# osmocom/osmo-trx

Measured on AMD Instinct MI355X. Metric: Mbursts/s detect+demod (156.25 sym, 4 SPS), higher is better.
Workload: dtype f32

## Files before the change

osmo_trx_amd/csrc/trx_kernel_nb.hip:

```cpp
#include "trx_k4_common.h"
#include "trx_nb_asm.inc"

#define NB_D_LEN    160
#define NB_CZ_LEN   (TRX_CZ_PAD + TRX_CORR_NARROW + TRX_CZ_PAD)
#define NB_SLICE    (K4_XS + NB_D_LEN + NB_CZ_LEN)
#define NB_COMP_ROWS (TRX_DELAY_FILTS + 1)
#define NB_TABLES_FLOATS (TRX_SINCV_LDS + 16 * WAVE + NB_COMP_ROWS * 36 + 16 + 8 * 8 + 5 * WAVE + 5 * WAVE + 2 * 8 * 16)
#define NB_TABLES_BYTES (NB_TABLES_FLOATS * 4)
#define NB_WPB 16
#define NB_POOL_RING 64
#define NB_POOL_UNSET (-1)
#define NB_POOL_END (-2)
#define NB_NO_BURST 0xffffffffu
#define NB_LDS_TAIL (16 + 4 * NB_POOL_RING)
#define NB_LDS_BYTES (NB_TABLES_BYTES + NB_WPB * NB_SLICE * 8 + NB_LDS_TAIL)
#define NB_MAX_TOA 32



typedef float v3f __attribute__((ext_vector_type(3)));
typedef int v4i __attribute__((ext_vector_type(4)));
typedef __attribute__((address_space(3))) v2f lds_v2f;

template <typename T>
__device__ __forceinline__ unsigned lds_addr(const T *p)
{
	return (unsigned)(uintptr_t)(const __attribute__((address_space(3))) T *)p;
}

__device__ __forceinline__ int nb_lane_id()
{
	int lane;
	asm volatile("v_mbcnt_lo_u32_b32 %0, -1, 0\n\tv_mbcnt_hi_u32_b32 %0, -1, %0" : "=v"(lane));
	return lane;
}

__global__ void __launch_bounds__(NB_WPB * WAVE)
nb_pull4_kernel(const uint32_t *__restrict__ iq, const trxhip_burst_params *__restrict__ params,
		trxhip_burst_result *__restrict__ results, float *__restrict__ soft, const trx_tables *__restrict__ tab,
		unsigned n_bursts, float thresh, float full_scale, unsigned *__restrict__ pool_ctr, unsigned *__restrict__ redo,
		float gk5, float gk6, float gk7, float gk8)
{
	static_assert(NB_TABLES_BYTES % 16 == 0 && (NB_SLICE * 8) % 16 == 0 && (K4_XS * 8) % 16 == 0 && (NB_D_LEN * 8) % 16 == 0, "16-byte LDS accesses");
	static_assert(NB_LDS_BYTES <= 160 * 1024, "LDS");
	static_assert(NB_ASM_GDEC_OFF == (TRX_SINCV_LDS + 16 * WAVE + NB_COMP_ROWS * 36) * 4, "tools/gen_nb_asm.py: LDS offset of the decimator taps");
	static_assert(NB_ASM_DEC_MAX_NACT == 15 + NB_ASM_CORR_MAX_LEN, "tools/gen_nb_asm.py: DEC and CORR change form at the same window (one test)");
	static_assert(NB_ASM_LSEQ_OFF == (NB_TABLES_FLOATS - 2 * 8 * 16) * 4, "tools/gen_nb_asm.py: LDS offset of the training-sequence taps");
	static_assert(NB_ASM_AW_PD == (PH_M0 + 52) * 8 && NB_ASM_AW_D == K4_XS * 8 && NB_ASM_AW_CZ == (K4_XS + NB_D_LEN + TRX_CZ_PAD) * 8,
		      "tools/gen_nb_asm.py: offsets of P, D[] and cz[] inside a wave's slice");
	constexpr int NLD = 10;
	extern __shared__ __attribute__((aligned(16))) char smem[];
	const int lane0 = threadIdx.x & (WAVE - 1);
	const int wave = uni((int)(threadIdx.x >> 6));

	float *const sincv = reinterpret_cast<float *>(smem);
	float *const wa4f = sincv + TRX_SINCV_LDS;
	const float4 *const wa4 = reinterpret_cast<const float4 *>(wa4f);
	float *const comp = wa4f + 16 * WAVE;
	float *const gdec = comp + NB_COMP_ROWS * 36;
	float *const lhdr = gdec + 16;
	int *const pkcl = reinterpret_cast<int *>(lhdr + 8 * 8);
	int *const lcn = pkcl + 5 * WAVE;
	c32 *const lseq = reinterpret_cast<c32 *>(lcn + 5 * WAVE);
	c32 *const wbase = reinterpret_cast<c32 *>(smem + NB_TABLES_BYTES) + (size_t)wave * NB_SLICE;
	int *const wg_next = reinterpret_cast<int *>(reinterpret_cast<c32 *>(smem + NB_TABLES_BYTES) + (size_t)NB_WPB * NB_SLICE);
	int *const pool_g = wg_next + 4;
	c32 *const P = wbase;
	c32 *const D = wbase + K4_XS;
	c32 *const cz = D + NB_D_LEN + TRX_CZ_PAD;

	for (int i = threadIdx.x; i < TRX_SINCV_LDS; i += blockDim.x)
		sincv[i] = (i < TRX_SINCV_LEN) ? tab->sincv[i] : 0.0f;
	for (int i = threadIdx.x; i < 16 * WAVE; i += blockDim.x) {
		const int l = i & (WAVE - 1), u = i >> 6;
		const PeakConst pcl = peak_const(l);
		const int q = (u < 8) ? pcl.loA + 512 * (7 - u) : pcl.hiA + 512 * (u - 8);
		wa4f[((u >> 2) * WAVE + l) * 4 + (u & 3)] = (q < TRX_SINCV_LEN) ? tab->sincv[q] : 0.0f;
	}
	for (int i = threadIdx.x; i < NB_COMP_ROWS * 36; i += blockDim.x) {
		const int f = i / 36, j = i % 36;
		comp[i] = (j >= TRX_FUSED_SH) ? tab->comp_filt[f][j - TRX_FUSED_SH] : 0.0f;
	}
	if (threadIdx.x < 16)
		gdec[threadIdx.x] = tab->dec_taps[threadIdx.x];
	if (threadIdx.x < 128)
		lseq[threadIdx.x] = make_float2(tab->seq[TRX_SEQ_TSC0 + (threadIdx.x >> 4)].taps[threadIdx.x & 15].re,
						tab->seq[TRX_SEQ_TSC0 + (threadIdx.x >> 4)].taps[threadIdx.x & 15].im);
	if (threadIdx.x < 64)
		lhdr[threadIdx.x] = reinterpret_cast<const float *>(&tab->seq[TRX_SEQ_TSC0 + (threadIdx.x >> 3)].gain)[threadIdx.x & 7];
	if (threadIdx.x < WAVE) {
		const PeakConst pc0 = peak_const(threadIdx.x);
		pkcl[0 * WAVE + threadIdx.x] = pc0.flA;
		pkcl[1 * WAVE + threadIdx.x] = pc0.loA;
		pkcl[2 * WAVE + threadIdx.x] = pc0.hiA;
		pkcl[3 * WAVE + threadIdx.x] = pc0.offB;
		pkcl[4 * WAVE + threadIdx.x] = pc0.ratio_off;
		lcn[0 * WAVE + threadIdx.x] = pc0.ratio_off * 8;
		lcn[1 * WAVE + threadIdx.x] = (pc0.flA - 8) * 8;
		lcn[2 * WAVE + threadIdx.x] = pc0.offB;
		const int l = threadIdx.x, e = (l - 52) / 3, t = (l - 52) % 3;
		const bool sp = l >= 52;
		lcn[3 * WAVE + l] = 8 * (sp ? (t == 0 ? e : t == 1 ? e + 3 : e - 3) : 4 + 3 * (l < 49 ? l : 49));
		lcn[4 * WAVE + l] = sp ? (e + (t == 2 ? 4 : 0)) * K4_NTP * 4 : -1;
	}
	for (int i = lane0; i < NB_SLICE; i += WAVE)
		wbase[i] = make_float2(0.0f, 0.0f);
	if (threadIdx.x == 0) {
		wg_next[0] = NB_WPB;
		wg_next[1] = 0;
	}
	if (threadIdx.x < NB_POOL_RING)
		pool_g[threadIdx.x] = NB_POOL_UNSET;
	__syncthreads();

	const float thr2 = thresh * thresh;
	float gkv = lane0 == 5 ? gk5 : lane0 == 6 ? gk6 : lane0 == 7 ? gk7 : gk8;
	asm volatile("" : "+v"(gkv));
	const float gc0 = thr2 * 1.0001e-5f;
	int t5pk = 0;
	bool t5_ok = true;
	for (int t = 0; t < 8; t++) {
		const int v = (int)(lhdr[8 * t + 5] * 512.0f);
		t5_ok = t5_ok && v >= -8 && v <= 7 && (float)v == lhdr[8 * t + 5] * 512.0f;
		t5pk |= (v & 15) << (4 * t);
	}
	t5pk = uni(t5pk);
	const unsigned toa_lim = (unsigned)uni(t5_ok ? (int)((NB_MAX_TOA + 1u) << 16) : 0);
	const unsigned long long e8_addr = reinterpret_cast<unsigned long long>(&tab->edge8[0][0][0]);
	const unsigned n_wg = gridDim.x;
	const unsigned n_groups = (n_bursts + 15u) >> 4;
	const bool pooled = pool_ctr != nullptr;
	const unsigned n_static_groups = pooled ? ((n_groups - (n_groups >> 3)) / n_wg) * n_wg : n_groups;
	const unsigned n_pool_groups = n_groups - n_static_groups;
	const unsigned gq = n_static_groups / n_wg, gr = n_static_groups % n_wg;
	const unsigned my_groups = gq + (blockIdx.x < gr ? 1u : 0u);
	const unsigned base16 = (blockIdx.x * gq + (blockIdx.x < gr ? blockIdx.x : gr)) << 4;
	unsigned items = my_groups << 4;
	if (base16 + items > n_bursts)
		items = (base16 < n_bursts) ? n_bursts - base16 : 0u;
	auto burst_of = [&](unsigned jj) -> unsigned {
		if (__builtin_expect(jj < items, 1))
			return base16 + jj;
		if (!pooled)
			return NB_NO_BURST;
		const unsigned k = (jj - items) >> 4;
		volatile int *slot = pool_g + (k & (NB_POOL_RING - 1));
		int g;
		while ((g = *slot) == NB_POOL_UNSET)
			__builtin_amdgcn_s_sleep(2);
		g = uni(g);
		if (g < 0)
			return NB_NO_BURST;
		const unsigned bb = ((n_static_groups + (unsigned)g) << 4) + (jj & 15u);
		return bb < n_bursts ? bb : NB_NO_BURST;
	};
	auto pool_draw = [&](unsigned jj, bool ended) {
		const int lane = nb_lane_id();
		const unsigned k = (jj + 16u - items) >> 4;
		int g = NB_POOL_END;
		if (!ended) {
			unsigned p = 0;
			if (lane == 0)
				p = __hip_atomic_fetch_add(pool_ctr, 1u, __ATOMIC_RELAXED, __HIP_MEMORY_SCOPE_AGENT);
			p = (unsigned)uni((int)p);
			g = (p < n_pool_groups) ? (int)p : NB_POOL_END;
		}
		if (lane == 0) {
			pool_g[(k + NB_POOL_RING / 2) & (NB_POOL_RING - 1)] = NB_POOL_UNSET;
			pool_g[k & (NB_POOL_RING - 1)] = g;
		}
	};

	unsigned a_p = lds_addr(wbase) + 8u * (unsigned)((lane0 & 3) * PH_A + PH_M0 + (lane0 >> 2));
	unsigned a_w = lds_addr(wbase) + 8u * (unsigned)lane0;
	unsigned a_l4 = 4u * (unsigned)lane0;
	unsigned a_l4c = 4u * min((unsigned)lane0, 48u);
	unsigned a_l16 = 16u * (unsigned)lane0;
	unsigned a_st = (lane0 >= 54) ? 4u * (unsigned)((lane0 - 54) / 3) : (unsigned)(lane0 - 2) * 12u + 16u;
	asm volatile("" : "+v"(a_p));
	asm volatile("" : "+v"(a_w));
	asm volatile("" : "+v"(a_l4));
	asm volatile("" : "+v"(a_l4c));
	asm volatile("" : "+v"(a_l16));
	asm volatile("" : "+v"(a_st));

	uint32_t pre_i[NLD];
	uint32_t pre_prm = 0u;
	auto prefetch = [&](unsigned bb) {
		pre_prm = reinterpret_cast<const uint32_t *>(params)[2 * (size_t)bb];
		const char *src = reinterpret_cast<const char *>(iq + (size_t)bb * 625);
		const uint32_t *const row = reinterpret_cast<const uint32_t *>(src + a_l4);
#pragma unroll
		for (int r = 0; r < NLD - 1; r++)
			pre_i[r] = __builtin_nontemporal_load(row + r * WAVE);
		pre_i[NLD - 1] = __builtin_nontemporal_load(reinterpret_cast<const uint32_t *>(src + a_l4c) + (NLD - 1) * WAVE);
	};
	const unsigned b_first = burst_of((unsigned)wave);
	if (b_first != NB_NO_BURST)
		prefetch(b_first);

	v3f o = { 0.0f, 0.0f, 0.0f };
	int recw = 0;
	int pend_m = 0;
	int pend_rm = 0;
	unsigned pend_b = 0;
	int left_any = 0;
	auto store_pending = [&]() {
		float *const so = soft + (size_t)pend_b * 148;
		int *const rp = reinterpret_cast<int *>(results + pend_b);
		const float oe = o.x;
		asm volatile("s_bfm_b64 exec, 48, 2\n\t"
			     "s_and_b32 exec_lo, exec_lo, %7\n\t"
			     "s_and_b32 exec_hi, exec_hi, %7\n\t"
			     "global_store_dwordx3 %0, %1, %2\n\t"
			     "s_mov_b32 exec_lo, 0\n\t"
			     "s_and_b32 exec_hi, %7, 0x92400000\n\t"
			     "global_store_dword %0, %3, %2\n\t"
			     "s_mov_b32 exec_lo, %8\n\t"
			     "s_mov_b32 exec_hi, 0\n\t"
			     "global_store_dword %4, %5, %6\n\t"
			     "s_mov_b64 exec, -1\n\t"
			     "s_nop 0"
			     :: "v"(a_st), "v"(o), "s"(so), "v"(oe), "v"(a_l4), "v"(recw), "s"(rp), "s"(pend_m), "s"(pend_rm)
			     : "memory", "scc");
	};
	int q_xr = 0, q_xi = 0, q_es = 0, q_toa = 0, q_s = 0, q_fl = 0, q_b = 0;
	int q_n = 0;
	auto flush_records = [&]() {
		const int lane = nb_lane_id();
		if (lane < q_n) {
			const float *const h = lhdr + 8 * (q_fl & 0xff);
			const float xr = __int_as_float(q_xr), xi = __int_as_float(q_xi);
			const float a0 = xr * h[2], a1 = xr * h[3], a2 = xi * h[3], a3 = xi * h[2];
			const float amp_re = a0 - a2, amp_im = a1 + a3;
			const float toa = (float)q_toa * 0.001953125f;
			const float energy = __int_as_float(q_es) * 0.0125f;
			const float rssi = rssi_db(full_scale, energy);
			const float p2 = xi * xi + xr * xr;
			const float C = p2 * h[7];
			const float S = __int_as_float(q_s);
			const float ci = 3.0103f * __log2f(C * __builtin_amdgcn_rcpf(S - C));
			const v4i r0 = { 1, __float_as_int(toa), __float_as_int(amp_re), __float_as_int(amp_im) };
			const v4i r1 = { __float_as_int(ci), __float_as_int(energy), __float_as_int(rssi), q_fl };
			asm volatile("global_store_dwordx4 %0, %1, off\n\t"
				     "global_store_dwordx4 %0, %2, off offset:16\n\t"
				     "s_nop 1"
				     :: "v"(results + (unsigned)q_b), "v"(r0), "v"(r1) : "memory");
		}
		asm volatile("");
		q_n = 0;
	};

	auto queue_record = [&](const int xr_bits, const int xi_bits, const int es_bits, const int toa, const int s_bits, const int fl, const unsigned bb) {
		asm("s_lshl_b64 exec, 1, %[n]\n\t"
		    "v_mov_b32_e32 %[qxr], %[xr]\n\t"
		    "v_mov_b32_e32 %[qxi], %[xi]\n\t"
		    "v_mov_b32_e32 %[qes], %[es]\n\t"
		    "v_mov_b32_e32 %[qtoa], %[toa]\n\t"
		    "v_mov_b32_e32 %[qs], %[ss]\n\t"
		    "v_mov_b32_e32 %[qfl], %[fl]\n\t"
		    "v_mov_b32_e32 %[qb], %[b]\n\t"
		    "s_mov_b64 exec, -1"
		    : [qxr] "+v"(q_xr), [qxi] "+v"(q_xi), [qes] "+v"(q_es), [qtoa] "+v"(q_toa), [qs] "+v"(q_s), [qfl] "+v"(q_fl),
		      [qb] "+v"(q_b)
		    : [n] "s"(uni(q_n)), [xr] "s"(xr_bits), [xi] "s"(xi_bits), [es] "s"(es_bits), [toa] "s"(toa),
		      [ss] "s"(s_bits), [fl] "s"(fl), [b] "s"((int)bb)
		    : "scc");
		q_n++;
	};

	auto demod_general = [&](const int nk, const c32 ampv, const int lane) -> bool {
		constexpr int L = 625, nwrite = 148;
		c32 *const dec = D;
		const trx_tables *tabc = reinterpret_cast<const trx_tables *>(e8_addr - offsetof(trx_tables, edge8));
		asm volatile("" : "+s"(tabc));
		const int w = nk >> 7, fr = nk & 127;
		const int fidx = (fr >= 2) ? (fr >> 1) : TRX_DELAY_FILTS;
		const float ian = __builtin_amdgcn_rcpf(norm2(ampv));
		const c32 scale = make_float2(ampv.x * ian, -ampv.y * ian);
		const int n_lo = w > 0 ? w : 0;
		const int n_hi = (L - 1 + w < 623) ? L - 1 + w : 623;
		const int i_full_lo = cdiv4(n_lo + 15), i_full_hi = fdiv4(n_hi);
		const int i0l = cdiv4(n_lo), i0h = i_full_hi + 1;
		const bool need_lo = (n_hi >= n_lo) && (i0l < i_full_lo) && (i0l < nwrite);
		const bool need_hi = (n_hi >= n_lo) && (i0h <= fdiv4(n_hi + 15)) && (i0h < nwrite);
		if (uni((need_lo && !(n_hi >= 4 * (i_full_lo - 1))) || (need_hi && !((w <= -2) && (n_lo <= 4 * i0h - 15)))))
			return false;
		const int lo_tab = uni(need_lo);
		float ct0 = 0.0f, ct1 = 0.0f, ct2 = 0.0f;
		const int le = lane >> 4, lt = lane & 15;
		const int li = i0l + le;
		const int lt0 = n_lo + 15 - 4 * li;
		const bool lact = lt0 >= 1;
		if (lo_tab) {
			const float *row = &tabc->edge_lo[fidx][(lact ? lt0 : 1) - 1][lt];
			ct0 = row[0];
			ct1 = row[16];
			ct2 = (lt < 4) ? row[32] : 0.0f;
		}
		const int hi_tab = uni(need_hi);
		float ch0 = 0.0f, ch1 = 0.0f, ch2 = 0.0f;
		const int hi_i = i0h + le;
		const int htm = n_hi + 15 - 4 * hi_i;
		const bool hact = htm >= 0;
		if (hi_tab) {
			const float *row = &tabc->edge_hi[fidx][hact ? htm : 0][lt];
			ch0 = row[0];
			ch1 = row[16];
			ch2 = (lt < 4) ? row[32] : 0.0f;
		}
		int tabv = lo_tab | (hi_tab << 1);
		asm volatile("" : "+v"(tabv));
		{
			const int c_full = -24 - w;
			const int i_min = cdiv4(-36 - c_full), i_max = fdiv4(L + 1 - c_full);
			int ic = 3 * lane;
			if (ic < i_min) ic = i_min;
			if (ic > i_max - 2) ic = i_max - 2;
			v2f acc[3];
			asm volatile(NB_ASM_FIRG
				     : [a0] "=&v"(acc[0]), [a1] "=&v"(acc[1]), [a2] "=&v"(acc[2])
				     : [nk] "s"(nk), [pb] "s"(lds_addr(P)), [cb] "s"(lds_addr(comp) + 4u * (K4_U0 + TRX_FUSED_SH)), [kic] "v"(8 * ic)
				     : NB_ASM_CLOBBERS);
			if (n_lo == 0 && lo_tab && i_full_hi >= nwrite - 1) {
				if (lane < 52) {
#pragma unroll
					for (int j = 0; j < 3; j++)
						dec[3 * lane + j] = cmul(make_float2(acc[j].x, acc[j].y), scale);
				}
			} else {
#pragma unroll
				for (int j = 0; j < 3; j++) {
					const int i = 3 * lane + j;
					const bool full = (i >= i_full_lo) && (i <= i_full_hi);
					const c32 d = full ? cmul(make_float2(acc[j].x, acc[j].y), scale) : make_float2(0.0f, 0.0f);
					if (i < 156)
						dec[i] = d;
				}
			}
		}
		const int tab2 = uni(tabv), lo_tab2 = tab2 & 1, hi_tab2 = tab2 & 2;
		if (lo_tab2) {
			const int s0 = 4 * li - 24 - w + lt;
			const c32 *pp = P + ((s0 & 3) * PH_A + PH_M0 + (s0 >> 2));
			const c32 x0 = lds_c32(pp), x1 = lds_c32(pp + 4), x2 = lds_c32(pp + 8);
			float ar = x0.x * ct0, ai = x0.y * ct0;
			ar = fmaf(x1.x, ct1, ar); ai = fmaf(x1.y, ct1, ai);
			ar = fmaf(x2.x, ct2, ar); ai = fmaf(x2.y, ct2, ai);
			const float sr = row_sum(ar), si = row_sum(ai);
			int lt0s = lt0;
			asm volatile("" : "+v"(lt0s));
			if (lt == 0 && lt0s >= 1)
				dec[li] = cmul(make_float2(sr, si), scale);
		}
		if (hi_tab2) {
			const int s0 = 4 * hi_i - 24 - w + lt;
			const c32 *pp = P + ((s0 & 3) * PH_A + PH_M0 + (s0 >> 2));
			const c32 x0 = lds_c32(pp), x1 = lds_c32(pp + 4), x2 = lds_c32(pp + 8);
			float ar = x0.x * ch0, ai = x0.y * ch0;
			ar = fmaf(x1.x, ch1, ar); ai = fmaf(x1.y, ch1, ai);
			ar = fmaf(x2.x, ch2, ar); ai = fmaf(x2.y, ch2, ai);
			const float sr = row_sum(ar), si = row_sum(ai);
			int htms = htm;
			asm volatile("" : "+v"(htms));
			if (lt == 0 && htms >= 0 && hi_i < 156)
				dec[hi_i] = cmul(make_float2(sr, si), scale);
		}
		wave_sync();
		auto pick = [&](int i) {
			const float d = reinterpret_cast<const float *>(dec + i)[i & 1];
			return __builtin_amdgcn_fmed3f(fmaf((i & 2) ? -0.5f : 0.5f, d, 0.5f), 0.0f, 1.0f);
		};
		const bool reg = lane >= 2 && lane < 50;
		const int i0 = reg ? 3 * lane - 2 : ((((lane - 54) * 11) >> 5) & 3);
		o.x = pick(i0);
		o.y = pick(reg ? i0 + 1 : 0);
		o.z = pick(reg ? i0 + 2 : 0);
		wave_sync();
		return true;
	};

	DIAG_DECL;
	unsigned j_next = 0, b_next = NB_NO_BURST;
	const unsigned j_plain = (unsigned)uni((int)(!pooled ? items : items >= 16u ? items - 16u : 0u));
	auto advance = [&](const int taken) {
		j_next = (unsigned)taken;
		if (__builtin_expect(j_next < j_plain, 1)) {
			b_next = base16 + j_next;
			DIAG_MARK(17);
			prefetch(b_next);
		} else {
			b_next = burst_of(j_next);
			if (pooled && (j_next & 15u) == 0u && j_next + 16u >= items)
				pool_draw(j_next, b_next == NB_NO_BURST && j_next >= items);
			DIAG_MARK(17);
			if (b_next != NB_NO_BURST)
				prefetch(b_next);
		}
	};
	auto mark_left = [&](const unsigned bb) {
		if (nb_lane_id() == 0) {
			reinterpret_cast<uint8_t *>(redo + TRX_REDO_HDR)[bb] = 1;
			if (!left_any)
				__hip_atomic_store(redo, 1u, __ATOMIC_RELAXED, __HIP_MEMORY_SCOPE_AGENT);
		}
		asm volatile("");
		left_any = 1;
	};
	for (unsigned b = b_first; __builtin_expect(b != NB_NO_BURST, 1); b = b_next) {
		asm volatile("" : "+v"(a_l4));
		asm volatile("" : "+v"(a_l4c));
		const int ticket = claim_issue(wg_next);
		const unsigned prm0 = (unsigned)uni((int)pre_prm);
		const unsigned max_toa = prm0 >> 16;
		const int tsc = (prm0 >> 8) & 0xff;
#ifdef TRX_DIAG
		DIAG_MARK(12);
		asm volatile("s_waitcnt vmcnt(0)" ::: "memory");
		DIAG_MARK(13);
#endif
		const unsigned slot_key = prm0 | (0u - ((prm0 & 0xf8ffu) ^ (unsigned)TRXHIP_TSC));
		int keep = -1;
		if (__builtin_expect(slot_key >= toa_lim, 0)) {
#pragma unroll
			for (int r = 0; r < NLD; r++)
				asm volatile("" :: "v"(pre_i[r]));
			store_pending();
			advance(claim_take(ticket));
			pend_rm = 0;
			mark_left(b);
			keep = 0;
		} else {
			lds_v2f *const pload = reinterpret_cast<lds_v2f *>(a_p);
			float amax = 0.0f, epart = 0.0f;
#pragma unroll
			for (int r = 0; r < NLD; r++) {
				const v2f v = { (float)(int16_t)(pre_i[r] & 0xffffu), (float)(int16_t)(pre_i[r] >> 16) };
				if (r < NLD - 1)
					pload[16 * r] = v;
				else
					asm volatile("s_bfm_b64 exec, 49, 0\n\t"
						     "ds_write_b64 %0, %1 offset:%c2\n\t"
						     "s_mov_b64 exec, -1"
						     :: "v"(a_p), "v"(v), "n"(128 * (NLD - 1)) : "memory");
				asm("v_max3_f32 %0, %0, |%1|, |%2|" : "+v"(amax) : "v"(v.x), "v"(v.y));
				if (r < 5)
					epart = fmaf(v.x, v.x, fmaf(v.y, v.y, epart));
			}
			DIAG_MARK(14);
			store_pending();
			DIAG_MARK(16);
			advance(claim_take_behind<5>(ticket));
			DIAG_MARK(15);

			pend_rm = 0;
			{
				int clip;
				asm("s_cmp_lg_u64 %1, 0\n\ts_cselect_b32 %0, 1, 0" : "=s"(clip) : "s"(__ballot(amax > TRX_CLIP_THRESH)) : "scc");

				const int len = 16 + (int)max_toa;
				__builtin_assume(len >= 16 && len <= 16 + NB_MAX_TOA);
				float v;
				const int lag0 = (len <= NB_ASM_CORR_MAX_LEN) ? NB_ASM_CORR_LANE0 : 0;
				asm volatile(NB_ASM_DECCORR
					     : [nrm] "=&v"(v)
					     : [aw] "v"(a_w), [zero] "v"(0), [len] "s"(len), [tsc] "s"(tsc)
					     : NB_ASM_CLOBBERS);
				{
					DIAG_MARK(3);
					int m_bits, es_bits, bidx;
					int kr, ka, kb, kic, ktp;
					asm volatile(NB_ASM_AMAX("ds_read_b32 %[kr], %[l4] offset:%c[lc]", "ds_read_b32 %[ka], %[l4] offset:%c[lc]+256",
								 "ds_read_b32 %[kb], %[l4] offset:%c[lc]+512", "ds_read_b32 %[kic], %[l4] offset:%c[lc]+768",
								 "ds_read_b32 %[ktp], %[l4] offset:%c[lc]+1024", "s_nop 0", "s_nop 0", "s_nop 0")
						     "s_sub_u32 %[bidx], %[bidx], %[lag0]\n\t"
						     "s_waitcnt lgkmcnt(0)"
						     : [m] "=&s"(m_bits), [es] "=&s"(es_bits), [bidx] "=&s"(bidx), [kr] "=&v"(kr), [ka] "=&v"(ka), [kb] "=&v"(kb),
						       [kic] "=&v"(kic), [ktp] "=&v"(ktp)
						     : [nrm] "v"(v), [ep] "v"(epart), [l4] "v"(a_l4), [lag0] "s"(lag0),
						       [lc] "n"((TRX_SINCV_LDS + 16 * WAVE + NB_COMP_ROWS * 36 + 16 + 64 + 5 * WAVE) * 4)
						     : NB_ASM_CLOBBERS);
					DIAG_MARK(4);
					int st, e512;
					float km;
					asm volatile(NB_ASM_DETA
						     : [st] "=&" NB_ASM_ST(st), [e] "=&s"(e512), [km] "=&v"(km)
						     : [bidx] "s"(bidx), [len] "s"(len), [czb] "s"(lds_addr(cz)), [kr] "v"(kr), [ka] "v"(ka), [l16] "v"(a_l16),
						       [gkv] "v"(gkv), [c0] "v"(gc0)
						     : NB_ASM_CLOBBERS_ST);
					DIAG_MARK(5);
					int toa512 = 0, xr_bits = 0, xi_bits = 0;
					if (__builtin_expect(st == 1, 1)) {
						asm volatile(NB_ASM_DETB
							     : [st] "=&" NB_ASM_ST(st), [toa] "=&s"(toa512), [xr] "=&s"(xr_bits), [xi] "=&s"(xi_bits)
							     : [e] "s"(e512), [kb] "v"(kb), [czb] "s"(lds_addr(cz)), [km] "v"(km)
							     : NB_ASM_CLOBBERS_ST);
						DIAG_MARK(6);
					}
					if (__builtin_expect(st != 1, 0)) {
						int stc = st;
						asm volatile("" : "+s"(stc));
						if (stc == 3) {
							const int lane = nb_lane_id();
							if (lane == 0)
								atomicAdd(&g_trx_fast_stats[0], 1ull);
							PeakConst pkc;
							pkc.flA = pkcl[0 * WAVE + lane]; pkc.loA = pkcl[1 * WAVE + lane]; pkc.hiA = pkcl[2 * WAVE + lane];
							pkc.offB = pkcl[3 * WAVE + lane]; pkc.ratio_off = pkcl[4 * WAVE + lane];
							c32 xcorr;
							peak_detect_spec(cz, bidx, sincv, pkc, lane, &toa512, &xcorr, wa4);
							toa512 = uni(toa512);
							xr_bits = uni(__float_as_int(xcorr.x));
							xi_bits = uni(__float_as_int(xcorr.y));
							st = 1;
						} else if (stc == 2) {
							if (nb_lane_id() == 0) atomicAdd(&g_trx_fast_stats[2], 1ull);
							mark_left(b);
							keep = 0;
						} else {
							const float energy = __int_as_float(es_bits) * 0.0125f;
							const float rssi = rssi_db(full_scale, energy);
							const uint32_t flags = ((uint32_t)clip << 8) | (1u << 16);
							int word = clip ? -TRXHIP_SIGERR_CLIP : 0;
							word = put_lane<1>(word, 0.0f);
							word = put_lane<2>(word, 0.0f);
							word = put_lane<3>(word, 0.0f);
							word = put_lane<4>(word, 0.0f);
							word = put_lane<5>(word, energy);
							word = put_lane<6>(word, rssi);
							word = write_lane<7>(word, (int)flags);
							recw = word;
							o = (v3f){ 0.0f, 0.0f, 0.0f };
							pend_rm = 0xff;
						}
					}
					if (__builtin_expect(st == 1, 1)) {
						int ok, s_bits;
						float d0, d1, d2;
						const int t5 = (t5pk << (28 - 4 * tsc)) >> 28;
						asm volatile("s_setprio 0");
						asm volatile(NB_ASM_TAIL
							     : [ok] "=&s"(ok), [ssum] "=&s"(s_bits), [d0] "=&v"(d0), [d1] "=&v"(d1), [d2] "=&v"(d2)
							     : [toa] "s"(toa512), [xr] "s"(xr_bits), [xi] "s"(xi_bits), [t5] "s"(t5), [hdrb] "s"(lds_addr(lhdr) + 32u * (unsigned)tsc),
							       [e8lo] "s"((unsigned)e8_addr), [e8hi] "s"((unsigned)(e8_addr >> 32)), [l16] "v"(a_l16),
							       [aw] "v"(a_w), [pb] "s"(lds_addr(P)), [cb] "s"(lds_addr(comp) + 4u * (K4_U0 + TRX_FUSED_SH)), [db] "s"(lds_addr(D)),
							       [kic] "v"(kic), [ktp] "v"(ktp)
							     : NB_ASM_CLOBBERS);
						DIAG_MARK(10);
						asm volatile("s_setprio 2");
						o.x = __builtin_amdgcn_fmed3f(fmaf(0.5f, d0, 0.5f), 0.0f, 1.0f);
						o.y = __builtin_amdgcn_fmed3f(fmaf(0.5f, d1, 0.5f), 0.0f, 1.0f);
						o.z = __builtin_amdgcn_fmed3f(fmaf(0.5f, d2, 0.5f), 0.0f, 1.0f);
						queue_record(xr_bits, xi_bits, es_bits, toa512 - t5 - 10 * 512, s_bits,
							     (int)((uint32_t)tsc | ((uint32_t)clip << 8) | (37u << 24)), b);
						if (__builtin_expect(!ok, 0)) {
							const int lane = nb_lane_id();
							if (lane == 0) atomicAdd(&g_trx_fast_stats[3], 1ull);
							const float *const h = lhdr + 8 * tsc;
							const float xr = __int_as_float(xr_bits), xi = __int_as_float(xi_bits);
							const float a0 = xr * h[2], a1 = xr * h[3], a2 = xi * h[3], a3 = xi * h[2];
							const c32 ampv = make_float2(unif(a0 - a2), unif(a1 + a3));
							if (!demod_general(t5 + 10 * 512 - toa512, ampv, lane)) {
								q_n--;
								mark_left(b);
								keep = 0;
							}
						}
					}
				}
			}
		}
		pend_b = b;
		pend_m = keep;
		if (__builtin_expect(q_n == WAVE, 0))
			flush_records();
		DIAG_MARK(11);
	}
	asm volatile(NB_ASM_COLD ::: NB_ASM_CLOBBERS);
	store_pending();
	flush_records();
	DIAG_FLUSH();
	if (pooled) {
		__syncthreads();
		int tid0;
		asm volatile("v_mbcnt_lo_u32_b32 %0, -1, 0\n\tv_mbcnt_hi_u32_b32 %0, -1, %0" : "=v"(tid0));
		if (tid0 == 0 && atomicAdd(wg_next + 1, 1) == 0) {
			const unsigned d = __hip_atomic_fetch_add(pool_ctr + 1, 1u, __ATOMIC_ACQ_REL, __HIP_MEMORY_SCOPE_AGENT);
			if (d == gridDim.x - 1u) {
				__hip_atomic_store(pool_ctr, 0u, __ATOMIC_RELAXED, __HIP_MEMORY_SCOPE_AGENT);
				__hip_atomic_store(pool_ctr + 1, 0u, __ATOMIC_RELEASE, __HIP_MEMORY_SCOPE_AGENT);
			}
		}
	}
}
```

osmo_trx_amd/csrc/trx_nb_asm.inc:

```
#define NB_ASM_GDEC_OFF 29968
#define NB_ASM_LSEQ_OFF 32848
#define NB_ASM_DEC_MAX_NACT 60
#define NB_ASM_CORR_LANE0 19
#define NB_ASM_CORR_MAX_LEN 45
#define NB_ASM_AW_PD 512
#define NB_ASM_AW_D 5760
#define NB_ASM_AW_CZ 7136
#define NB_ASM_ST "{s98}"
#define NB_ASM_CLOBBERS "v64", "v65", "v66", "v67", "v68", "v69", "v70", "v71", "v72", "v73", "v74", "v75", "v76", "v77", "v78", "v79", "v80", "v81", "v82", "v83", "v84", "v85", "v86", "v87", "v88", "v89", "v90", "v91", "v92", "v93", "v94", "v95", "v96", "v97", "v98", "v99", "v100", "v101", "v102", "v103", "v104", "v105", "v106", "v107", "v108", "v109", "v110", "v111", "v112", "v113", "v114", "v115", "v116", "v117", "v118", "v119", "v120", "v121", "v122", "v123", "v124", "v125", "v126", "v127", "s87", "s88", "s89", "s90", "s91", "s92", "s93", "s94", "s95", "s96", "s97", "s98", "s99", "vcc", "scc", "memory"
#define NB_ASM_CLOBBERS_ST "v64", "v65", "v66", "v67", "v68", "v69", "v70", "v71", "v72", "v73", "v74", "v75", "v76", "v77", "v78", "v79", "v80", "v81", "v82", "v83", "v84", "v85", "v86", "v87", "v88", "v89", "v90", "v91", "v92", "v93", "v94", "v95", "v96", "v97", "v98", "v99", "v100", "v101", "v102", "v103", "v104", "v105", "v106", "v107", "v108", "v109", "v110", "v111", "v112", "v113", "v114", "v115", "v116", "v117", "v118", "v119", "v120", "v121", "v122", "v123", "v124", "v125", "v126", "v127", "s87", "s88", "s89", "s90", "s91", "s92", "s93", "s94", "s95", "s96", "s97", "s99", "vcc", "scc", "memory"
#define NB_ASM_DECCORR \
	"s_add_u32 s92, %[len], 15\n\t" \
	"s_cmp_gt_u32 %[len], 45\n\t" \
	"s_cbranch_scc1 .Lnbc_dc_wide\n\t" \
	"s_sub_u32 s88, 60, s92\n\t" \
	"s_lshr_b64 exec, -1, s88\n\t" \
	"ds_read_b128 v[120:123], %[zero] offset:29968\n\t" \
	"ds_read_b128 v[124:127], %[zero] offset:29984\n\t" \
	"ds_read_b64 v[98:99], %[aw] offset:1952\n\t" \
	"ds_read_b64 v[100:101], %[aw] offset:3392\n\t" \
	"ds_read_b64 v[102:103], %[aw] offset:4832\n\t" \
	"ds_read_b64 v[96:97], %[aw] offset:512\n\t" \
	"s_waitcnt lgkmcnt(3)\n\t" \
	"v_pk_mul_f32 v[64:65], v[98:99], v[120:121] op_sel:[0,0] op_sel_hi:[1,0]\n\t" \
// ... 880 lines not shown
	"v_add_f32_dpp v121, v121, v110 wave_shr:1 row_mask:0xf bank_mask:0xf bound_ctrl:0\n\t" \
	"s_nop 0\n\t" \
	"v_add_f32_dpp v120, v120, v110 wave_shr:1 row_mask:0xf bank_mask:0xf bound_ctrl:0\n\t" \
	"v_add_f32_dpp v121, v121, v111 wave_shr:1 row_mask:0xf bank_mask:0xf bound_ctrl:0\n\t" \
	"s_nop 0\n\t" \
	"v_sub_f32_dpp v120, v120, v111 wave_shr:1 row_mask:0xf bank_mask:0xf bound_ctrl:0\n\t" \
	"v_add_f32_dpp v121, v121, v110 wave_shr:1 row_mask:0xf bank_mask:0xf bound_ctrl:0\n\t" \
	"s_nop 0\n\t" \
	"v_sub_f32_dpp v120, v120, v110 wave_shr:1 row_mask:0xf bank_mask:0xf bound_ctrl:0\n\t" \
	"v_sub_f32_dpp v121, v121, v111 wave_shr:1 row_mask:0xf bank_mask:0xf bound_ctrl:0\n\t" \
	"s_nop 0\n\t" \
	"v_add_f32_dpp v120, v120, v111 wave_shr:1 row_mask:0xf bank_mask:0xf bound_ctrl:0\n\t" \
	"v_sub_f32_dpp v121, v121, v110 wave_shr:1 row_mask:0xf bank_mask:0xf bound_ctrl:0\n\t" \
	"s_nop 0\n\t" \
	"v_sub_f32_dpp v120, v120, v110 wave_shr:1 row_mask:0xf bank_mask:0xf bound_ctrl:0\n\t" \
	"v_sub_f32_dpp v121, v121, v111 wave_shr:1 row_mask:0xf bank_mask:0xf bound_ctrl:0\n\t" \
	"s_nop 0\n\t" \
	"v_sub_f32_dpp v120, v120, v111 wave_shr:1 row_mask:0xf bank_mask:0xf bound_ctrl:0\n\t" \
	"v_add_f32_dpp v121, v121, v110 wave_shr:1 row_mask:0xf bank_mask:0xf bound_ctrl:0\n\t" \
	"s_nop 0\n\t" \
	"v_sub_f32_dpp v120, v120, v110 wave_shr:1 row_mask:0xf bank_mask:0xf bound_ctrl:0\n\t" \
	"v_sub_f32_dpp v121, v121, v111 wave_shr:1 row_mask:0xf bank_mask:0xf bound_ctrl:0\n\t" \
	"s_nop 0\n\t" \
	"v_add_f32_dpp v120, v120, v111 wave_shr:1 row_mask:0xf bank_mask:0xf bound_ctrl:0\n\t" \
	"v_sub_f32_dpp v121, v121, v110 wave_shr:1 row_mask:0xf bank_mask:0xf bound_ctrl:0\n\t" \
	"s_nop 0\n\t" \
	"v_sub_f32_dpp v120, v120, v110 wave_shr:1 row_mask:0xf bank_mask:0xf bound_ctrl:0\n\t" \
	"v_sub_f32_dpp v121, v121, v111 wave_shr:1 row_mask:0xf bank_mask:0xf bound_ctrl:0\n\t" \
	"s_nop 0\n\t" \
	"v_sub_f32_dpp v120, v120, v111 wave_shr:1 row_mask:0xf bank_mask:0xf bound_ctrl:0\n\t" \
	"v_add_f32_dpp v121, v121, v110 wave_shr:1 row_mask:0xf bank_mask:0xf bound_ctrl:0\n\t" \
	"s_bfm_b64 exec, 12, 0\n\t" \
	"ds_write_b64 v64, v[122:123] offset:7136\n\t" \
	"s_bfm_b64 exec, %[len], 19\n\t" \
	"ds_write_b64 %[aw], v[120:121] offset:6984\n\t" \
	"v_pk_mul_f32 v[124:125], v[120:121], v[120:121]\n\t" \
	"s_nop 0\n\t" \
	"v_add_f32_e32 %[nrm], v125, v124\n\t" \
	"s_mov_b64 exec, -1\n\t" \
	"s_waitcnt lgkmcnt(0)\n\t" \
	"s_branch .Lnb_corr_end\n\t" \
	".Lnb_corrr_v4:\n\t" \
	"v_add_f32_e32 v120, 0, v110\n\t" \
	"v_add_f32_e32 v121, 0, v111\n\t" \
	"s_nop 0\n\t" \
	"v_sub_f32_dpp v120, v120, v111 wave_shr:1 row_mask:0xf bank_mask:0xf bound_ctrl:0\n\t" \
	"v_add_f32_dpp v121, v121, v110 wave_shr:1 row_mask:0xf bank_mask:0xf bound_ctrl:0\n\t" \
	"s_nop 0\n\t" \
	"v_sub_f32_dpp v120, v120, v110 wave_shr:1 row_mask:0xf bank_mask:0xf bound_ctrl:0\n\t" \
	"v_sub_f32_dpp v121, v121, v111 wave_shr:1 row_mask:0xf bank_mask:0xf bound_ctrl:0\n\t" \
	"s_nop 0\n\t" \
	"v_add_f32_dpp v120, v120, v111 wave_shr:1 row_mask:0xf bank_mask:0xf bound_ctrl:0\n\t" \
	"v_sub_f32_dpp v121, v121, v110 wave_shr:1 row_mask:0xf bank_mask:0xf bound_ctrl:0\n\t" \
	"s_nop 0\n\t" \
	"v_sub_f32_dpp v120, v120, v110 wave_shr:1 row_mask:0xf bank_mask:0xf bound_ctrl:0\n\t" \
	"v_sub_f32_dpp v121, v121, v111 wave_shr:1 row_mask:0xf bank_mask:0xf bound_ctrl:0\n\t" \
	"s_nop 0\n\t" \
	"v_sub_f32_dpp v120, v120, v111 wave_shr:1 row_mask:0xf bank_mask:0xf bound_ctrl:0\n\t" \
	"v_add_f32_dpp v121, v121, v110 wave_shr:1 row_mask:0xf bank_mask:0xf bound_ctrl:0\n\t" \
	"s_nop 0\n\t" \
	"v_sub_f32_dpp v120, v120, v110 wave_shr:1 row_mask:0xf bank_mask:0xf bound_ctrl:0\n\t" \
	"v_sub_f32_dpp v121, v121, v111 wave_shr:1 row_mask:0xf bank_mask:0xf bound_ctrl:0\n\t" \
	"s_nop 0\n\t" \
	"v_sub_f32_dpp v120, v120, v111 wave_shr:1 row_mask:0xf bank_mask:0xf bound_ctrl:0\n\t" \
	"v_add_f32_dpp v121, v121, v110 wave_shr:1 row_mask:0xf bank_mask:0xf bound_ctrl:0\n\t" \
	"s_nop 0\n\t" \
	"v_sub_f32_dpp v120, v120, v110 wave_shr:1 row_mask:0xf bank_mask:0xf bound_ctrl:0\n\t" \
	"v_sub_f32_dpp v121, v121, v111 wave_shr:1 row_mask:0xf bank_mask:0xf bound_ctrl:0\n\t" \
	"s_nop 0\n\t" \
	"v_add_f32_dpp v120, v120, v111 wave_shr:1 row_mask:0xf bank_mask:0xf bound_ctrl:0\n\t" \
	"v_sub_f32_dpp v121, v121, v110 wave_shr:1 row_mask:0xf bank_mask:0xf bound_ctrl:0\n\t" \
	"s_nop 0\n\t" \
	"v_sub_f32_dpp v120, v120, v110 wave_shr:1 row_mask:0xf bank_mask:0xf bound_ctrl:0\n\t" \
	"v_sub_f32_dpp v121, v121, v111 wave_shr:1 row_mask:0xf bank_mask:0xf bound_ctrl:0\n\t" \
	"s_nop 0\n\t" \
	"v_sub_f32_dpp v120, v120, v111 wave_shr:1 row_mask:0xf bank_mask:0xf bound_ctrl:0\n\t" \
	"v_add_f32_dpp v121, v121, v110 wave_shr:1 row_mask:0xf bank_mask:0xf bound_ctrl:0\n\t" \
	"s_nop 0\n\t" \
	"v_add_f32_dpp v120, v120, v110 wave_shr:1 row_mask:0xf bank_mask:0xf bound_ctrl:0\n\t" \
	"v_add_f32_dpp v121, v121, v111 wave_shr:1 row_mask:0xf bank_mask:0xf bound_ctrl:0\n\t" \
	"s_nop 0\n\t" \
	"v_add_f32_dpp v120, v120, v111 wave_shr:1 row_mask:0xf bank_mask:0xf bound_ctrl:0\n\t" \
	"v_sub_f32_dpp v121, v121, v110 wave_shr:1 row_mask:0xf bank_mask:0xf bound_ctrl:0\n\t" \
	"s_nop 0\n\t" \
	"v_add_f32_dpp v120, v120, v110 wave_shr:1 row_mask:0xf bank_mask:0xf bound_ctrl:0\n\t" \
	"v_add_f32_dpp v121, v121, v111 wave_shr:1 row_mask:0xf bank_mask:0xf bound_ctrl:0\n\t" \
	"s_nop 0\n\t" \
	"v_add_f32_dpp v120, v120, v111 wave_shr:1 row_mask:0xf bank_mask:0xf bound_ctrl:0\n\t" \
	"v_sub_f32_dpp v121, v121, v110 wave_shr:1 row_mask:0xf bank_mask:0xf bound_ctrl:0\n\t" \
	"s_bfm_b64 exec, 12, 0\n\t" \
	"ds_write_b64 v64, v[122:123] offset:7136\n\t" \
	"s_bfm_b64 exec, %[len], 19\n\t" \
	"ds_write_b64 %[aw], v[120:121] offset:6984\n\t" \
	"v_pk_mul_f32 v[124:125], v[120:121], v[120:121]\n\t" \
	"s_nop 0\n\t" \
	"v_add_f32_e32 %[nrm], v125, v124\n\t" \
	"s_mov_b64 exec, -1\n\t" \
	"s_waitcnt lgkmcnt(0)\n\t" \
	"s_branch .Lnb_corr_end\n\t" \
	".Lnb_corrr_v5:\n\t" \
	"v_sub_f32_e32 v120, 0, v110\n\t" \
	"v_sub_f32_e32 v121, 0, v111\n\t" \
	"s_nop 0\n\t" \
	"v_sub_f32_dpp v120, v120, v111 wave_shr:1 row_mask:0xf bank_mask:0xf bound_ctrl:0\n\t" \
	"v_add_f32_dpp v121, v121, v110 wave_shr:1 row_mask:0xf bank_mask:0xf bound_ctrl:0\n\t" \
	"s_nop 0\n\t" \
	"v_sub_f32_dpp v120, v120, v110 wave_shr:1 row_mask:0xf bank_mask:0xf bound_ctrl:0\n\t" \
	"v_sub_f32_dpp v121, v121, v111 wave_shr:1 row_mask:0xf bank_mask:0xf bound_ctrl:0\n\t" \
	"s_nop 0\n\t" \
	"v_add_f32_dpp v120, v120, v111 wave_shr:1 row_mask:0xf bank_mask:0xf bound_ctrl:0\n\t" \
	"v_sub_f32_dpp v121, v121, v110 wave_shr:1 row_mask:0xf bank_mask:0xf bound_ctrl:0\n\t" \
	"s_nop 0\n\t" \
	"v_add_f32_dpp v120, v120, v110 wave_shr:1 row_mask:0xf bank_mask:0xf bound_ctrl:0\n\t" \
	"v_add_f32_dpp v121, v121, v111 wave_shr:1 row_mask:0xf bank_mask:0xf bound_ctrl:0\n\t" \
	"s_nop 0\n\t" \
	"v_sub_f32_dpp v120, v120, v111 wave_shr:1 row_mask:0xf bank_mask:0xf bound_ctrl:0\n\t" \
	"v_add_f32_dpp v121, v121, v110 wave_shr:1 row_mask:0xf bank_mask:0xf bound_ctrl:0\n\t" \
	"s_nop 0\n\t" \
	"v_add_f32_dpp v120, v120, v110 wave_shr:1 row_mask:0xf bank_mask:0xf bound_ctrl:0\n\t" \
	"v_add_f32_dpp v121, v121, v111 wave_shr:1 row_mask:0xf bank_mask:0xf bound_ctrl:0\n\t" \
	"s_nop 0\n\t" \
	"v_sub_f32_dpp v120, v120, v111 wave_shr:1 row_mask:0xf bank_mask:0xf bound_ctrl:0\n\t" \
	"v_add_f32_dpp v121, v121, v110 wave_shr:1 row_mask:0xf bank_mask:0xf bound_ctrl:0\n\t" \
	"s_nop 0\n\t" \
	"v_add_f32_dpp v120, v120, v110 wave_shr:1 row_mask:0xf bank_mask:0xf bound_ctrl:0\n\t" \
	"v_add_f32_dpp v121, v121, v111 wave_shr:1 row_mask:0xf bank_mask:0xf bound_ctrl:0\n\t" \
	"s_nop 0\n\t" \
	"v_add_f32_dpp v120, v120, v111 wave_shr:1 row_mask:0xf bank_mask:0xf bound_ctrl:0\n\t" \
	"v_sub_f32_dpp v121, v121, v110 wave_shr:1 row_mask:0xf bank_mask:0xf bound_ctrl:0\n\t" \
	"s_nop 0\n\t" \
	"v_sub_f32_dpp v120, v120, v110 wave_shr:1 row_mask:0xf bank_mask:0xf bound_ctrl:0\n\t" \
	"v_sub_f32_dpp v121, v121, v111 wave_shr:1 row_mask:0xf bank_mask:0xf bound_ctrl:0\n\t" \
	"s_nop 0\n\t" \
	"v_sub_f32_dpp v120, v120, v111 wave_shr:1 row_mask:0xf bank_mask:0xf bound_ctrl:0\n\t" \
	"v_add_f32_dpp v121, v121, v110 wave_shr:1 row_mask:0xf bank_mask:0xf bound_ctrl:0\n\t" \
	"s_nop 0\n\t" \
	"v_sub_f32_dpp v120, v120, v110 wave_shr:1 row_mask:0xf bank_mask:0xf bound_ctrl:0\n\t" \
	"v_sub_f32_dpp v121, v121, v111 wave_shr:1 row_mask:0xf bank_mask:0xf bound_ctrl:0\n\t" \
	"s_nop 0\n\t" \
	"v_add_f32_dpp v120, v120, v111 wave_shr:1 row_mask:0xf bank_mask:0xf bound_ctrl:0\n\t" \
	"v_sub_f32_dpp v121, v121, v110 wave_shr:1 row_mask:0xf bank_mask:0xf bound_ctrl:0\n\t" \
	"s_nop 0\n\t" \
	"v_sub_f32_dpp v120, v120, v110 wave_shr:1 row_mask:0xf bank_mask:0xf bound_ctrl:0\n\t" \
	"v_sub_f32_dpp v121, v121, v111 wave_shr:1 row_mask:0xf bank_mask:0xf bound_ctrl:0\n\t" \
	"s_nop 0\n\t" \
	"v_add_f32_dpp v120, v120, v111 wave_shr:1 row_mask:0xf bank_mask:0xf bound_ctrl:0\n\t" \
	"v_sub_f32_dpp v121, v121, v110 wave_shr:1 row_mask:0xf bank_mask:0xf bound_ctrl:0\n\t" \
	"s_bfm_b64 exec, 12, 0\n\t" \
	"ds_write_b64 v64, v[122:123] offset:7136\n\t" \
	"s_bfm_b64 exec, %[len], 19\n\t" \
	"ds_write_b64 %[aw], v[120:121] offset:6984\n\t" \
	"v_pk_mul_f32 v[124:125], v[120:121], v[120:121]\n\t" \
	"s_nop 0\n\t" \
	"v_add_f32_e32 %[nrm], v125, v124\n\t" \
	"s_mov_b64 exec, -1\n\t" \
	"s_waitcnt lgkmcnt(0)\n\t" \
	"s_branch .Lnb_corr_end\n\t" \
	".Lnb_corrr_v6:\n\t" \
	"v_sub_f32_e32 v120, 0, v110\n\t" \
	"v_sub_f32_e32 v121, 0, v111\n\t" \
	"s_nop 0\n\t" \
	"v_sub_f32_dpp v120, v120, v111 wave_shr:1 row_mask:0xf bank_mask:0xf bound_ctrl:0\n\t" \
	"v_add_f32_dpp v121, v121, v110 wave_shr:1 row_mask:0xf bank_mask:0xf bound_ctrl:0\n\t" \
	"s_nop 0\n\t" \
	"v_add_f32_dpp v120, v120, v110 wave_shr:1 row_mask:0xf bank_mask:0xf bound_ctrl:0\n\t" \
	"v_add_f32_dpp v121, v121, v111 wave_shr:1 row_mask:0xf bank_mask:0xf bound_ctrl:0\n\t" \
	"s_nop 0\n\t" \
	"v_add_f32_dpp v120, v120, v111 wave_shr:1 row_mask:0xf bank_mask:0xf bound_ctrl:0\n\t" \
	"v_sub_f32_dpp v121, v121, v110 wave_shr:1 row_mask:0xf bank_mask:0xf bound_ctrl:0\n\t" \
	"s_nop 0\n\t" \
	"v_sub_f32_dpp v120, v120, v110 wave_shr:1 row_mask:0xf bank_mask:0xf bound_ctrl:0\n\t" \
	"v_sub_f32_dpp v121, v121, v111 wave_shr:1 row_mask:0xf bank_mask:0xf bound_ctrl:0\n\t" \
	"s_nop 0\n\t" \
	"v_add_f32_dpp v120, v120, v111 wave_shr:1 row_mask:0xf bank_mask:0xf bound_ctrl:0\n\t" \
	"v_sub_f32_dpp v121, v121, v110 wave_shr:1 row_mask:0xf bank_mask:0xf bound_ctrl:0\n\t" \
	"s_nop 0\n\t" \
	"v_add_f32_dpp v120, v120, v110 wave_shr:1 row_mask:0xf bank_mask:0xf bound_ctrl:0\n\t" \
	"v_add_f32_dpp v121, v121, v111 wave_shr:1 row_mask:0xf bank_mask:0xf bound_ctrl:0\n\t" \
	"s_nop 0\n\t" \
	"v_add_f32_dpp v120, v120, v111 wave_shr:1 row_mask:0xf bank_mask:0xf bound_ctrl:0\n\t" \
	"v_sub_f32_dpp v121, v121, v110 wave_shr:1 row_mask:0xf bank_mask:0xf bound_ctrl:0\n\t" \
	"s_nop 0\n\t" \
	"v_add_f32_dpp v120, v120, v110 wave_shr:1 row_mask:0xf bank_mask:0xf bound_ctrl:0\n\t" \
	"v_add_f32_dpp v121, v121, v111 wave_shr:1 row_mask:0xf bank_mask:0xf bound_ctrl:0\n\t" \
	"s_nop 0\n\t" \
	"v_add_f32_dpp v120, v120, v111 wave_shr:1 row_mask:0xf bank_mask:0xf bound_ctrl:0\n\t" \
	"v_sub_f32_dpp v121, v121, v110 wave_shr:1 row_mask:0xf bank_mask:0xf bound_ctrl:0\n\t" \
	"s_nop 0\n\t" \
	"v_sub_f32_dpp v120, v120, v110 wave_shr:1 row_mask:0xf bank_mask:0xf bound_ctrl:0\n\t" \
	"v_sub_f32_dpp v121, v121, v111 wave_shr:1 row_mask:0xf bank_mask:0xf bound_ctrl:0\n\t" \
	"s_nop 0\n\t" \
	"v_add_f32_dpp v120, v120, v111 wave_shr:1 row_mask:0xf bank_mask:0xf bound_ctrl:0\n\t" \
	"v_sub_f32_dpp v121, v121, v110 wave_shr:1 row_mask:0xf bank_mask:0xf bound_ctrl:0\n\t" \
	"s_nop 0\n\t" \
	"v_add_f32_dpp v120, v120, v110 wave_shr:1 row_mask:0xf bank_mask:0xf bound_ctrl:0\n\t" \
	"v_add_f32_dpp v121, v121, v111 wave_shr:1 row_mask:0xf bank_mask:0xf bound_ctrl:0\n\t" \
	"s_nop 0\n\t" \
	"v_sub_f32_dpp v120, v120, v111 wave_shr:1 row_mask:0xf bank_mask:0xf bound_ctrl:0\n\t" \
	"v_add_f32_dpp v121, v121, v110 wave_shr:1 row_mask:0xf bank_mask:0xf bound_ctrl:0\n\t" \
	"s_nop 0\n\t" \
	"v_sub_f32_dpp v120, v120, v110 wave_shr:1 row_mask:0xf bank_mask:0xf bound_ctrl:0\n\t" \
	"v_sub_f32_dpp v121, v121, v111 wave_shr:1 row_mask:0xf bank_mask:0xf bound_ctrl:0\n\t" \
	"s_nop 0\n\t" \
	"v_sub_f32_dpp v120, v120, v111 wave_shr:1 row_mask:0xf bank_mask:0xf bound_ctrl:0\n\t" \
	"v_add_f32_dpp v121, v121, v110 wave_shr:1 row_mask:0xf bank_mask:0xf bound_ctrl:0\n\t" \
	"s_bfm_b64 exec, 12, 0\n\t" \
	"ds_write_b64 v64, v[122:123] offset:7136\n\t" \
	"s_bfm_b64 exec, %[len], 19\n\t" \
	"ds_write_b64 %[aw], v[120:121] offset:6984\n\t" \
	"v_pk_mul_f32 v[124:125], v[120:121], v[120:121]\n\t" \
	"s_nop 0\n\t" \
	"v_add_f32_e32 %[nrm], v125, v124\n\t" \
	"s_mov_b64 exec, -1\n\t" \
	"s_waitcnt lgkmcnt(0)\n\t" \
	"s_branch .Lnb_corr_end\n\t" \
	".Lnb_corrr_v7:\n\t" \
	"v_sub_f32_e32 v120, 0, v110\n\t" \
	"v_sub_f32_e32 v121, 0, v111\n\t" \
	"s_nop 0\n\t" \
	"v_sub_f32_dpp v120, v120, v111 wave_shr:1 row_mask:0xf bank_mask:0xf bound_ctrl:0\n\t" \
	"v_add_f32_dpp v121, v121, v110 wave_shr:1 row_mask:0xf bank_mask:0xf bound_ctrl:0\n\t" \
	"s_nop 0\n\t" \
	"v_add_f32_dpp v120, v120, v110 wave_shr:1 row_mask:0xf bank_mask:0xf bound_ctrl:0\n\t" \
	"v_add_f32_dpp v121, v121, v111 wave_shr:1 row_mask:0xf bank_mask:0xf bound_ctrl:0\n\t" \
	"s_nop 0\n\t" \
	"v_sub_f32_dpp v120, v120, v111 wave_shr:1 row_mask:0xf bank_mask:0xf bound_ctrl:0\n\t" \
	"v_add_f32_dpp v121, v121, v110 wave_shr:1 row_mask:0xf bank_mask:0xf bound_ctrl:0\n\t" \
	"s_nop 0\n\t" \
	"v_add_f32_dpp v120, v120, v110 wave_shr:1 row_mask:0xf bank_mask:0xf bound_ctrl:0\n\t" \
	"v_add_f32_dpp v121, v121, v111 wave_shr:1 row_mask:0xf bank_mask:0xf bound_ctrl:0\n\t" \
	"s_nop 0\n\t" \
	"v_add_f32_dpp v120, v120, v111 wave_shr:1 row_mask:0xf bank_mask:0xf bound_ctrl:0\n\t" \
	"v_sub_f32_dpp v121, v121, v110 wave_shr:1 row_mask:0xf bank_mask:0xf bound_ctrl:0\n\t" \
	"s_nop 0\n\t" \
	"v_add_f32_dpp v120, v120, v110 wave_shr:1 row_mask:0xf bank_mask:0xf bound_ctrl:0\n\t" \
	"v_add_f32_dpp v121, v121, v111 wave_shr:1 row_mask:0xf bank_mask:0xf bound_ctrl:0\n\t" \
	"s_nop 0\n\t" \
	"v_sub_f32_dpp v120, v120, v111 wave_shr:1 row_mask:0xf bank_mask:0xf bound_ctrl:0\n\t" \
	"v_add_f32_dpp v121, v121, v110 wave_shr:1 row_mask:0xf bank_mask:0xf bound_ctrl:0\n\t" \
	"s_nop 0\n\t" \
	"v_add_f32_dpp v120, v120, v110 wave_shr:1 row_mask:0xf bank_mask:0xf bound_ctrl:0\n\t" \
	"v_add_f32_dpp v121, v121, v111 wave_shr:1 row_mask:0xf bank_mask:0xf bound_ctrl:0\n\t" \
	"s_nop 0\n\t" \
	"v_sub_f32_dpp v120, v120, v111 wave_shr:1 row_mask:0xf bank_mask:0xf bound_ctrl:0\n\t" \
	"v_add_f32_dpp v121, v121, v110 wave_shr:1 row_mask:0xf bank_mask:0xf bound_ctrl:0\n\t" \
	"s_nop 0\n\t" \
	"v_sub_f32_dpp v120, v120, v110 wave_shr:1 row_mask:0xf bank_mask:0xf bound_ctrl:0\n\t" \
	"v_sub_f32_dpp v121, v121, v111 wave_shr:1 row_mask:0xf bank_mask:0xf bound_ctrl:0\n\t" \
	"s_nop 0\n\t" \
	"v_add_f32_dpp v120, v120, v111 wave_shr:1 row_mask:0xf bank_mask:0xf bound_ctrl:0\n\t" \
	"v_sub_f32_dpp v121, v121, v110 wave_shr:1 row_mask:0xf bank_mask:0xf bound_ctrl:0\n\t" \
	"s_nop 0\n\t" \
	"v_sub_f32_dpp v120, v120, v110 wave_shr:1 row_mask:0xf bank_mask:0xf bound_ctrl:0\n\t" \
	"v_sub_f32_dpp v121, v121, v111 wave_shr:1 row_mask:0xf bank_mask:0xf bound_ctrl:0\n\t" \
	"s_nop 0\n\t" \
	"v_sub_f32_dpp v120, v120, v111 wave_shr:1 row_mask:0xf bank_mask:0xf bound_ctrl:0\n\t" \
	"v_add_f32_dpp v121, v121, v110 wave_shr:1 row_mask:0xf bank_mask:0xf bound_ctrl:0\n\t" \
	"s_nop 0\n\t" \
	"v_sub_f32_dpp v120, v120, v110 wave_shr:1 row_mask:0xf bank_mask:0xf bound_ctrl:0\n\t" \
	"v_sub_f32_dpp v121, v121, v111 wave_shr:1 row_mask:0xf bank_mask:0xf bound_ctrl:0\n\t" \
	"s_nop 0\n\t" \
	"v_add_f32_dpp v120, v120, v111 wave_shr:1 row_mask:0xf bank_mask:0xf bound_ctrl:0\n\t" \
	"v_sub_f32_dpp v121, v121, v110 wave_shr:1 row_mask:0xf bank_mask:0xf bound_ctrl:0\n\t" \
	"s_bfm_b64 exec, 12, 0\n\t" \
	"ds_write_b64 v64, v[122:123] offset:7136\n\t" \
	"s_bfm_b64 exec, %[len], 19\n\t" \
	"ds_write_b64 %[aw], v[120:121] offset:6984\n\t" \
	"v_pk_mul_f32 v[124:125], v[120:121], v[120:121]\n\t" \
	"s_nop 0\n\t" \
	"v_add_f32_e32 %[nrm], v125, v124\n\t" \
	"s_mov_b64 exec, -1\n\t" \
	"s_waitcnt lgkmcnt(0)\n\t" \
	".Lnb_corr_end:\n\t"
#define NB_ASM_DETA \
	"s_mov_b32 s98, 0\n\t" \
	"s_sub_u32 s88, %[bidx], 3\n\t" \
	"s_sub_u32 s89, %[len], 6\n\t" \
	"s_cmp_gt_u32 s88, s89\n\t" \
	"s_cbranch_scc1 .Lnb_da_end\n\t" \
	"s_lshl3_add_u32 s89, %[bidx], %[czb]\n\t" \
	"s_add_u32 s90, %[len], -1\n\t" \
	"v_mov_b32_e32 v64, s89\n\t" \
	"v_add_u32_e32 v65, s89, %[kr]\n\t" \
	"s_lshl3_add_u32 s90, s90, %[czb]\n\t" \
	"v_add_u32_e32 v66, s89, %[ka]\n\t" \
	"ds_read_b64 v[68:69], v64\n\t" \
	"v_mov_b32_e32 v67, s90\n\t" \
	"v_mov_b64_e32 v[72:73], 0\n\t" \
	"s_bfm_b64 exec, 8, 0\n\t" \
	"ds_read_b64 v[70:71], v65\n\t" \
	"s_mov_b64 exec, 1\n\t" \
	"ds_write_b64 v67, v[72:73]\n\t" \
	"s_mov_b64 exec, -1\n\t" \
	"ds_read_b128 v[76:79], %[l16] offset:16512\n\t" \
	"ds_read_b128 v[80:83], %[l16] offset:17536\n\t" \
	"ds_read_b64 v[88:89], v66 offset:0\n\t" \
	"ds_read_b64 v[90:91], v66 offset:8\n\t" \
	"ds_read_b64 v[92:93], v66 offset:16\n\t" \
	"ds_read_b64 v[94:95], v66 offset:24\n\t" \
	"ds_read_b64 v[96:97], v66 offset:32\n\t" \
	"ds_read_b64 v[98:99], v66 offset:40\n\t" \
	"ds_read_b64 v[100:101], v66 offset:48\n\t" \
	"ds_read_b64 v[102:103], v66 offset:56\n\t" \
	"v_mov_b64_e32 v[84:85], 0\n\t" \
	"v_mov_b64_e32 v[86:87], 0\n\t" \
	"s_add_u32 s91, %[bidx], -1\n\t" \
	"s_sub_u32 s92, %[len], %[bidx]\n\t" \
	"s_min_u32 s91, s91, 4\n\t" \
	"s_waitcnt lgkmcnt(11)\n\t" \
	"v_pk_mul_f32 v[68:69], v[68:69], v[68:69]\n\t" \
	"s_add_u32 s92, s92, -2\n\t" \
	"v_add_f32_e32 v74, v69, v68\n\t" \
	"v_mul_f32_e32 %[km], 0x36c9539c, v74\n\t" \
	"s_bfm_b64 exec, 8, 0\n\t" \
	"v_pk_mul_f32 v[70:71], v[70:71], v[70:71]\n\t" \
	"s_min_u32 s92, s92, 4\n\t" \
	"v_add_f32_e32 v75, v71, v70\n\t" \
	"s_add_u32 s91, s91, s92\n\t" \
	"v_readlane_b32 s92, %[gkv], s91\n\t" \
	"v_add_f32_dpp v75, v75, v75 quad_perm:[1,0,3,2] row_mask:0xf bank_mask:0xf\n\t" \
	"s_nop 1\n\t" \
	"v_add_f32_dpp v75, v75, v75 quad_perm:[2,3,0,1] row_mask:0xf bank_mask:0xf\n\t" \
	"s_nop 1\n\t" \
	"v_add_f32_dpp v75, v75, v75 row_half_mirror row_mask:0xf bank_mask:0xf\n\t" \
	"v_mul_f32_e32 v112, s92, v75\n\t" \
	"v_mul_f32_e32 v113, 0x3f7fff37, v112\n\t" \
	"v_fmamk_f32 v114, v112, 0x3f8000c9, %[c0]\n\t" \
	"v_cmp_gt_f32_e32 vcc, v74, v114\n\t" \
	"s_cbranch_vccz .Lnbc_da_gate\n\t" \
	"s_mov_b64 exec, -1\n\t" \
	"ds_read_b128 v[104:107], %[l16] offset:18560\n\t" \
	"ds_read_b128 v[108:111], %[l16] offset:19584\n\t" \
	"ds_read_b64 v[112:113], v66 offset:64\n\t" \
	"ds_read_b64 v[114:115], v66 offset:72\n\t" \
	"ds_read_b64 v[116:117], v66 offset:80\n\t" \
	"ds_read_b64 v[118:119], v66 offset:88\n\t" \
	"ds_read_b64 v[120:121], v66 offset:96\n\t" \
	"ds_read_b64 v[122:123], v66 offset:104\n\t" \
	"ds_read_b64 v[124:125], v66 offset:112\n\t" \
	"ds_read_b64 v[126:127], v66 offset:120\n\t" \
	"s_waitcnt lgkmcnt(10)\n\t" \
	"v_pk_fma_f32 v[84:85], v[88:89], v[76:77], v[84:85] op_sel:[0,0,0] op_sel_hi:[1,0,1]\n\t" \
	"v_pk_fma_f32 v[86:87], v[90:91], v[76:77], v[86:87] op_sel:[0,1,0] op_sel_hi:[1,1,1]\n\t" \
	"v_pk_fma_f32 v[84:85], v[92:93], v[78:79], v[84:85] op_sel:[0,0,0] op_sel_hi:[1,0,1]\n\t" \
	"v_pk_fma_f32 v[86:87], v[94:95], v[78:79], v[86:87] op_sel:[0,1,0] op_sel_hi:[1,1,1]\n\t" \
	"v_pk_fma_f32 v[84:85], v[96:97], v[80:81], v[84:85] op_sel:[0,0,0] op_sel_hi:[1,0,1]\n\t" \
	"v_pk_fma_f32 v[86:87], v[98:99], v[80:81], v[86:87] op_sel:[0,1,0] op_sel_hi:[1,1,1]\n\t" \
	"v_pk_fma_f32 v[84:85], v[100:101], v[82:83], v[84:85] op_sel:[0,0,0] op_sel_hi:[1,0,1]\n\t" \
	"v_pk_fma_f32 v[86:87], v[102:103], v[82:83], v[86:87] op_sel:[0,1,0] op_sel_hi:[1,1,1]\n\t" \
	"s_waitcnt lgkmcnt(0)\n\t" \
	"v_pk_fma_f32 v[84:85], v[112:113], v[104:105], v[84:85] op_sel:[0,0,0] op_sel_hi:[1,0,1]\n\t" \
	"v_pk_fma_f32 v[86:87], v[114:115], v[104:105], v[86:87] op_sel:[0,1,0] op_sel_hi:[1,1,1]\n\t" \
	"v_pk_fma_f32 v[84:85], v[116:117], v[106:107], v[84:85] op_sel:[0,0,0] op_sel_hi:[1,0,1]\n\t" \
	"v_pk_fma_f32 v[86:87], v[118:119], v[106:107], v[86:87] op_sel:[0,1,0] op_sel_hi:[1,1,1]\n\t" \
	"v_pk_fma_f32 v[84:85], v[120:121], v[108:109], v[84:85] op_sel:[0,0,0] op_sel_hi:[1,0,1]\n\t" \
	"v_pk_fma_f32 v[86:87], v[122:123], v[108:109], v[86:87] op_sel:[0,1,0] op_sel_hi:[1,1,1]\n\t" \
	"v_pk_fma_f32 v[84:85], v[124:125], v[110:111], v[84:85] op_sel:[0,0,0] op_sel_hi:[1,0,1]\n\t" \
	"v_pk_fma_f32 v[86:87], v[126:127], v[110:111], v[86:87] op_sel:[0,1,0] op_sel_hi:[1,1,1]\n\t" \
	"s_nop 0\n\t" \
	"v_pk_add_f32 v[84:85], v[84:85], v[86:87]\n\t" \
	"s_nop 0\n\t" \
	"v_pk_mul_f32 v[84:85], v[84:85], v[84:85]\n\t" \
	"s_nop 0\n\t" \
	"v_add_f32_e32 v88, v85, v84\n\t" \
	"v_fmamk_f32 v89, v88, 0x36c9539c, %[km]\n\t" \
	"v_sub_f32_e32 v90, v88, v89\n\t" \
	"v_add_f32_e32 v91, v88, v89\n\t" \
	"s_lshl_b32 s94, %[bidx], 9\n\t" \
	"v_mov_b32_dpp v90, v90 quad_perm:[1,0,3,2] row_mask:0xf bank_mask:0xf\n\t" \
	"v_cmp_lt_f32_e64 s[88:89], v91, v90\n\t" \
	"s_mov_b32 s98, 1\n\t" \
	"s_lshr_b64 s[90:91], s[88:89], 1\n\t" \
	"s_or_b64 s[90:91], s[90:91], s[88:89]\n\t" \
	"s_mov_b32 s96, 0x55555555\n\t" \
	"s_mov_b32 s97, 0x15555555\n\t" \
	"s_and_b64 s[92:93], s[90:91], s[96:97]\n\t" \
	"s_cmp_eq_u64 s[92:93], s[96:97]\n\t" \
	"s_cbranch_scc0 .Lnbc_da_careful\n\t" \
	"s_mov_b32 s95, 0\n\t" \
	"s_lshl1_add_u32 s96, s95, 0\n\t" \
	"s_bitcmp1_b64 s[88:89], s96\n\t" \
	"s_addc_u32 s95, s95, s95\n\t" \
	"s_lshl1_add_u32 s96, s95, 2\n\t" \
	"s_bitcmp1_b64 s[88:89], s96\n\t" \
	"s_addc_u32 s95, s95, s95\n\t" \
	"s_lshl1_add_u32 s96, s95, 6\n\t" \
	"s_bitcmp1_b64 s[88:89], s96\n\t" \
	"s_addc_u32 s95, s95, s95\n\t" \
	"s_lshl1_add_u32 s96, s95, 14\n\t" \
	"s_bitcmp1_b64 s[88:89], s96\n\t" \
	"s_addc_u32 s95, s95, s95\n\t" \
	"s_lshl1_add_u32 s96, s95, 30\n\t" \
	"s_bitcmp1_b64 s[88:89], s96\n\t" \
	"s_addc_u32 s95, s95, s95\n\t" \
	".Lnb_da_walked:\n\t" \
	"s_lshl_b32 s95, s95, 5\n\t" \
	"s_add_u32 s94, s94, s95\n\t" \
	"s_add_u32 %[e], s94, -1008\n\t" \
	".Lnb_da_end:\n\t"
#define NB_ASM_DETB \
	"v_mov_b64_e32 v[64:65], 0\n\t" \
	"v_mov_b64_e32 v[66:67], 0\n\t" \
	"v_add_u32_e32 v68, %[e], %[kb]\n\t" \
	"s_add_u32 s88, %[czb], -56\n\t" \
	"s_mov_b32 exec_lo, 0x3fffffff\n\t" \
	"s_mov_b32 exec_hi, 0xffff\n\t" \
	"v_ashrrev_i32_e32 v69, 9, v68\n\t" \
	"v_and_b32_e32 v70, 0x1ff, v68\n\t" \
	"v_lshl_add_u32 v69, v69, 3, s88\n\t" \
	"v_bfe_u32 v71, v70, 4, 5\n\t" \
	"v_sub_u32_e32 v72, 0x200, v70\n\t" \
	"v_xor_b32_e32 v71, v71, v70\n\t" \
	"v_bfe_u32 v73, v72, 4, 5\n\t" \
	"v_lshlrev_b32_e32 v71, 2, v71\n\t" \
	"v_xor_b32_e32 v72, v73, v72\n\t" \
	"v_lshlrev_b32_e32 v72, 2, v72\n\t" \
	"ds_read_b64 v[80:81], v69 offset:0\n\t" \
	"ds_read_b32 v96, v71 offset:14336\n\t" \
	"ds_read_b64 v[82:83], v69 offset:8\n\t" \
	"ds_read_b32 v97, v71 offset:12288\n\t" \
	"ds_read_b64 v[84:85], v69 offset:16\n\t" \
	"ds_read_b32 v98, v71 offset:10240\n\t" \
	"ds_read_b64 v[86:87], v69 offset:24\n\t" \
	"ds_read_b32 v99, v71 offset:8192\n\t" \
	"ds_read_b64 v[88:89], v69 offset:32\n\t" \
	"ds_read_b32 v100, v71 offset:6144\n\t" \
	"ds_read_b64 v[90:91], v69 offset:40\n\t" \
	"ds_read_b32 v101, v71 offset:4096\n\t" \
	"ds_read_b64 v[92:93], v69 offset:48\n\t" \
	"ds_read_b32 v102, v71 offset:2048\n\t" \
	"ds_read_b64 v[94:95], v69 offset:56\n\t" \
	"ds_read_b32 v103, v71 offset:0\n\t" \
	"s_waitcnt lgkmcnt(12)\n\t" \
	"v_pk_fma_f32 v[64:65], v[80:81], v[96:97], v[64:65] op_sel:[0,0,0] op_sel_hi:[1,0,1]\n\t" \
	"v_pk_fma_f32 v[66:67], v[82:83], v[96:97], v[66:67] op_sel:[0,1,0] op_sel_hi:[1,1,1]\n\t" \
	"ds_read_b64 v[104:105], v69 offset:64\n\t" \
	"ds_read_b32 v120, v72 offset:0\n\t" \
	"ds_read_b64 v[106:107], v69 offset:72\n\t" \
	"ds_read_b32 v121, v72 offset:2048\n\t" \
	"s_waitcnt lgkmcnt(12)\n\t" \
	"v_pk_fma_f32 v[64:65], v[84:85], v[98:99], v[64:65] op_sel:[0,0,0] op_sel_hi:[1,0,1]\n\t" \
	"v_pk_fma_f32 v[66:67], v[86:87], v[98:99], v[66:67] op_sel:[0,1,0] op_sel_hi:[1,1,1]\n\t" \
	"ds_read_b64 v[108:109], v69 offset:80\n\t" \
	"ds_read_b32 v122, v72 offset:4096\n\t" \
	"ds_read_b64 v[110:111], v69 offset:88\n\t" \
	"ds_read_b32 v123, v72 offset:6144\n\t" \
	"s_waitcnt lgkmcnt(12)\n\t" \
	"v_pk_fma_f32 v[64:65], v[88:89], v[100:101], v[64:65] op_sel:[0,0,0] op_sel_hi:[1,0,1]\n\t" \
	"v_pk_fma_f32 v[66:67], v[90:91], v[100:101], v[66:67] op_sel:[0,1,0] op_sel_hi:[1,1,1]\n\t" \
	"ds_read_b64 v[112:113], v69 offset:96\n\t" \
	"ds_read_b32 v124, v72 offset:8192\n\t" \
	"ds_read_b64 v[114:115], v69 offset:104\n\t" \
	"ds_read_b32 v125, v72 offset:10240\n\t" \
	"s_waitcnt lgkmcnt(12)\n\t" \
	"v_pk_fma_f32 v[64:65], v[92:93], v[102:103], v[64:65] op_sel:[0,0,0] op_sel_hi:[1,0,1]\n\t" \
	"v_pk_fma_f32 v[66:67], v[94:95], v[102:103], v[66:67] op_sel:[0,1,0] op_sel_hi:[1,1,1]\n\t" \
	"ds_read_b64 v[116:117], v69 offset:112\n\t" \
	"ds_read_b32 v126, v72 offset:12288\n\t" \
	"ds_read_b64 v[118:119], v69 offset:120\n\t" \
	"ds_read_b32 v127, v72 offset:14336\n\t" \
	"s_waitcnt lgkmcnt(12)\n\t" \
	"v_pk_fma_f32 v[64:65], v[104:105], v[120:121], v[64:65] op_sel:[0,0,0] op_sel_hi:[1,0,1]\n\t" \
	"v_pk_fma_f32 v[66:67], v[106:107], v[120:121], v[66:67] op_sel:[0,1,0] op_sel_hi:[1,1,1]\n\t" \
	"s_waitcnt lgkmcnt(8)\n\t" \
	"v_pk_fma_f32 v[64:65], v[108:109], v[122:123], v[64:65] op_sel:[0,0,0] op_sel_hi:[1,0,1]\n\t" \
	"v_pk_fma_f32 v[66:67], v[110:111], v[122:123], v[66:67] op_sel:[0,1,0] op_sel_hi:[1,1,1]\n\t" \
	"s_waitcnt lgkmcnt(4)\n\t" \
	"v_pk_fma_f32 v[64:65], v[112:113], v[124:125], v[64:65] op_sel:[0,0,0] op_sel_hi:[1,0,1]\n\t" \
	"v_pk_fma_f32 v[66:67], v[114:115], v[124:125], v[66:67] op_sel:[0,1,0] op_sel_hi:[1,1,1]\n\t" \
	"s_waitcnt lgkmcnt(0)\n\t" \
	"v_pk_fma_f32 v[64:65], v[116:117], v[126:127], v[64:65] op_sel:[0,0,0] op_sel_hi:[1,0,1]\n\t" \
	"v_pk_fma_f32 v[66:67], v[118:119], v[126:127], v[66:67] op_sel:[0,1,0] op_sel_hi:[1,1,1]\n\t" \
	"s_mov_b64 exec, -1\n\t" \
	"v_pk_add_f32 v[74:75], v[64:65], v[66:67]\n\t" \
	"s_add_u32 s92, %[e], 497\n\t" \
	"v_pk_mul_f32 v[76:77], v[74:75], v[74:75]\n\t" \
	"s_mov_b32 s98, 1\n\t" \
	"v_add_f32_e32 v78, v77, v76\n\t" \
	"v_fmamk_f32 v79, v78, 0x36c9539c, %[km]\n\t" \
	"v_sub_f32_e32 v96, v78, v79\n\t" \
	"v_add_f32_e32 v97, v78, v79\n\t" \
	"s_nop 0\n\t" \
	"v_mov_b32_dpp v96, v96 quad_perm:[1,0,3,2] row_mask:0xf bank_mask:0xf\n\t" \
	"v_cmp_lt_f32_e64 s[88:89], v97, v96\n\t" \
	"s_lshr_b32 s90, s88, 1\n\t" \
	"s_or_b32 s90, s90, s88\n\t" \
	"s_and_b32 s91, s90, 0x15555555\n\t" \
	"s_cmp_eq_u32 s91, 0x15555555\n\t" \
	"s_cbranch_scc0 .Lnbc_db_careful\n\t" \
	"s_mov_b32 s94, 0\n\t" \
	"s_lshl1_add_u32 s95, s94, 0\n\t" \
	"s_bitcmp1_b32 s88, s95\n\t" \
	"s_addc_u32 s94, s94, s94\n\t" \
	"s_lshl1_add_u32 s95, s94, 2\n\t" \
	"s_bitcmp1_b32 s88, s95\n\t" \
	"s_addc_u32 s94, s94, s94\n\t" \
	"s_lshl1_add_u32 s95, s94, 6\n\t" \
	"s_bitcmp1_b32 s88, s95\n\t" \
	"s_addc_u32 s94, s94, s94\n\t" \
	"s_lshl1_add_u32 s95, s94, 14\n\t" \
	"s_bitcmp1_b32 s88, s95\n\t" \
	"s_addc_u32 s94, s94, s94\n\t" \
	".Lnb_db_walked:\n\t" \
	"s_add_u32 s93, s94, 32\n\t" \
	"s_lshl1_add_u32 %[toa], s94, s92\n\t" \
	"v_readlane_b32 %[xr], v74, s93\n\t" \
	"v_readlane_b32 %[xi], v75, s93\n\t" \
	".Lnb_db_end:\n\t"
#define NB_ASM_TAIL \
	"v_mov_b32_e32 v65, %[hdrb]\n\t" \
	"ds_read_b128 v[68:71], v65\n\t" \
	"s_sub_u32 s88, %[t5], %[toa]\n\t" \
	"s_add_u32 s87, s88, 5120\n\t" \
	"s_mov_b32 %[ok], 0\n\t" \
	"s_and_b32 s91, s87, 127\n\t" \
	"s_lshr_b32 s92, s91, 1\n\t" \
	"s_cmp_ge_u32 s91, 2\n\t" \
	"s_cselect_b32 s92, s92, 64\n\t" \
	"s_mul_i32 s93, s92, 768\n\t" \
	"s_add_u32 s94, %[e8lo], s93\n\t" \
	"s_addc_u32 s95, %[e8hi], 0\n\t" \
	"s_abs_i32 s96, %[toa]\n\t" \
	"s_add_u32 s96, s96, 256\n\t" \
	"global_load_dwordx4 v[120:123], %[l16], s[94:95]\n\t" \
	"s_lshr_b32 s96, s96, 9\n\t" \
	"s_sub_u32 s97, 0, s96\n\t" \
	"s_cmp_lt_i32 %[toa], 0\n\t" \
	"s_cselect_b32 s96, s97, s96\n\t" \
	"s_lshl_b32 s96, s96, 3\n\t" \
	"v_add_u32_e32 v64, s96, %[aw]\n\t" \
	"s_bfm_b64 exec, 16, 0\n\t" \
	"ds_read_b64 v[66:67], v64 offset:5760\n\t" \
	"s_mov_b64 exec, -1\n\t" \
	"s_waitcnt lgkmcnt(1)\n\t" \
	"v_mul_f32_e32 v82, %[xr], v70\n\t" \
	"v_mul_f32_e32 v83, %[xr], v71\n\t" \
	"v_mul_f32_e32 v84, %[xi], v71\n\t" \
	"v_mul_f32_e32 v85, %[xi], v70\n\t" \
	"v_sub_f32_e32 v86, v82, v84\n\t" \
	"v_add_f32_e32 v87, v83, v85\n\t" \
	"v_mul_f32_e32 v90, v86, v86\n\t" \
	"v_mul_f32_e32 v89, v87, v87\n\t" \
	"v_add_f32_e32 v89, v89, v90\n\t" \
	"v_rcp_f32_e32 v89, v89\n\t" \
	"s_mov_b32 s88, 0xaaaaaaaa\n\t" \
	"s_mov_b32 s89, 0xaaaaaaaa\n\t" \
	"v_mul_f32_e32 v91, v86, v89\n\t" \
	"v_mul_f32_e64 v92, -v87, v89\n\t" \
	"v_cndmask_b32_e64 v119, v91, v92, s[88:89]\n\t" \
	"s_mov_b32 s88, 0xcccccccc\n\t" \
	"s_mov_b32 s89, 0xcccccccc\n\t" \
	"v_cndmask_b32_e64 v119, v119, -v119, s[88:89]\n\t" \
	"s_bfm_b64 exec, 16, 0\n\t" \
	"s_waitcnt lgkmcnt(0)\n\t" \
	"v_pk_mul_f32 v[66:67], v[66:67], v[66:67]\n\t" \
	"s_ashr_i32 s88, s87, 7\n\t" \
	"v_add_f32_e32 v81, v67, v66\n\t" \
	"s_and_b32 s89, s87, 127\n\t" \
	"s_lshr_b32 s90, s89, 1\n\t" \
	"v_add_f32_dpp v81, v81, v81 quad_perm:[1,0,3,2] row_mask:0xf bank_mask:0xf\n\t" \
	"s_cmp_ge_u32 s89, 2\n\t" \
	"s_cselect_b32 s90, s90, 64\n\t" \
	"v_add_f32_dpp v81, v81, v81 quad_perm:[2,3,0,1] row_mask:0xf bank_mask:0xf\n\t" \
	"s_sub_u32 s91, -18, s88\n\t" \
	"s_and_b32 s92, s91, 3\n\t" \
	"v_add_f32_dpp v81, v81, v81 row_half_mirror row_mask:0xf bank_mask:0xf\n\t" \
	"s_ashr_i32 s93, s91, 2\n\t" \
	"s_mul_i32 s94, s92, 180\n\t" \
	"v_add_f32_dpp v81, v81, v81 row_mirror row_mask:0xf bank_mask:0xf\n\t" \
	"s_add_u32 s94, s94, s93\n\t" \
	"s_lshl3_add_u32 s94, s94, %[pb]\n\t" \
	"v_mul_f32_e32 v81, 0x3d800000, v81\n\t" \
	"s_mul_i32 s95, s90, 144\n\t" \
	"s_add_u32 s95, s95, %[cb]\n\t" \
	"v_readlane_b32 %[ssum], v81, 0\n\t" \
	"s_mov_b64 exec, -1\n\t" \
	"s_sub_u32 s96, 0, s88\n\t" \
	"s_cmp_gt_u32 s96, 36\n\t" \
	"s_cbranch_scc1 .Lnbc_tl_wait\n\t" \
	"s_mov_b32 %[ok], 1\n\t" \
	"v_add_u32_e32 v112, s94, %[kic]\n\t" \
	"s_add_u32 s96, s92, 1\n\t" \
	"s_lshr_b32 s96, s96, 2\n\t" \
	"s_mul_i32 s96, s96, -5752\n\t" \
	"s_add_u32 s96, s96, 1440\n\t" \
	"v_add_u32_e32 v113, s96, v112\n\t" \
	"s_add_u32 s96, s92, 2\n\t" \
	"s_lshr_b32 s96, s96, 2\n\t" \
	"s_mul_i32 s96, s96, -5752\n\t" \
	"s_add_u32 s96, s96, 2880\n\t" \
	"v_add_u32_e32 v114, s96, v112\n\t" \
	"s_add_u32 s96, s92, 3\n\t" \
	"s_lshr_b32 s96, s96, 2\n\t" \
	"s_mul_i32 s96, s96, -5752\n\t" \
	"s_add_u32 s96, s96, 4320\n\t" \
	"v_add_u32_e32 v115, s96, v112\n\t" \
	"ds_read_b64 v[72:73], v112 offset:96\n\t" \
	"ds_read_b64 v[74:75], v113 offset:96\n\t" \
	"ds_read_b64 v[76:77], v114 offset:96\n\t" \
	"ds_read_b64 v[78:79], v115 offset:96\n\t" \
	"ds_read_b64 v[80:81], v112 offset:104\n\t" \
	"ds_read_b64 v[82:83], v113 offset:104\n\t" \
	"ds_read_b64 v[84:85], v114 offset:104\n\t" \
	"ds_read_b64 v[86:87], v115 offset:104\n\t" \
	"ds_read_b64 v[88:89], v112 offset:112\n\t" \
	"ds_read_b64 v[90:91], v113 offset:112\n\t" \
	"ds_read_b64 v[92:93], v114 offset:112\n\t" \
	"ds_read_b64 v[94:95], v115 offset:112\n\t" \
	"v_add_u32_e32 v116, %[db], %[l16]\n\t" \
	"v_cmp_lt_i32_e32 vcc, -1, %[ktp]\n\t" \
	"v_add_u32_e32 v117, %[db], %[ktp]\n\t" \
	"v_mov_b32_e32 v118, s95\n\t" \
	"v_mov_b64_e32 v[64:65], 0\n\t" \
	"v_mov_b64_e32 v[66:67], 0\n\t" \
	"v_mov_b64_e32 v[68:69], 0\n\t" \
	"v_cndmask_b32_e32 v117, v118, v117, vcc\n\t" \
	"s_waitcnt vmcnt(0)\n\t" \
	"ds_write_b128 v116, v[120:123]\n\t" \
	"ds_read_b128 v[96:99], v117 offset:0\n\t" \
	"ds_read_b128 v[100:103], v117 offset:16\n\t" \
	"ds_read_b128 v[104:107], v117 offset:32\n\t" \
	"ds_read_b128 v[108:111], v117 offset:48\n\t" \
	"ds_read_b128 v[124:127], v117 offset:64\n\t" \
	"s_waitcnt lgkmcnt(4)\n\t" \
	"ds_read_b128 v[120:123], v117 offset:80\n\t" \
	"v_pk_fma_f32 v[64:65], v[72:73], v[96:97], v[64:65] op_sel:[0,0,0] op_sel_hi:[1,0,1]\n\t" \
	"v_pk_fma_f32 v[66:67], v[80:81], v[96:97], v[66:67] op_sel:[0,0,0] op_sel_hi:[1,0,1]\n\t" \
	"v_pk_fma_f32 v[68:69], v[88:89], v[96:97], v[68:69] op_sel:[0,0,0] op_sel_hi:[1,0,1]\n\t" \
	"v_pk_fma_f32 v[64:65], v[74:75], v[96:97], v[64:65] op_sel:[0,1,0] op_sel_hi:[1,1,1]\n\t" \
	"v_pk_fma_f32 v[66:67], v[82:83], v[96:97], v[66:67] op_sel:[0,1,0] op_sel_hi:[1,1,1]\n\t" \
	"v_pk_fma_f32 v[68:69], v[90:91], v[96:97], v[68:69] op_sel:[0,1,0] op_sel_hi:[1,1,1]\n\t" \
	"v_pk_fma_f32 v[64:65], v[76:77], v[98:99], v[64:65] op_sel:[0,0,0] op_sel_hi:[1,0,1]\n\t" \
	"v_pk_fma_f32 v[66:67], v[84:85], v[98:99], v[66:67] op_sel:[0,0,0] op_sel_hi:[1,0,1]\n\t" \
	"v_pk_fma_f32 v[68:69], v[92:93], v[98:99], v[68:69] op_sel:[0,0,0] op_sel_hi:[1,0,1]\n\t" \
	"v_pk_fma_f32 v[64:65], v[78:79], v[98:99], v[64:65] op_sel:[0,1,0] op_sel_hi:[1,1,1]\n\t" \
	"v_pk_fma_f32 v[66:67], v[86:87], v[98:99], v[66:67] op_sel:[0,1,0] op_sel_hi:[1,1,1]\n\t" \
	"v_pk_fma_f32 v[68:69], v[94:95], v[98:99], v[68:69] op_sel:[0,1,0] op_sel_hi:[1,1,1]\n\t" \
	"s_waitcnt lgkmcnt(4)\n\t" \
	"v_pk_fma_f32 v[64:65], v[80:81], v[100:101], v[64:65] op_sel:[0,0,0] op_sel_hi:[1,0,1]\n\t" \
	"v_pk_fma_f32 v[66:67], v[88:89], v[100:101], v[66:67] op_sel:[0,0,0] op_sel_hi:[1,0,1]\n\t" \
	"v_mov_b32_dpp v68, v68 wave_shr:1 row_mask:0xf bank_mask:0xf bound_ctrl:0\n\t" \
	"v_mov_b32_dpp v69, v69 wave_shr:1 row_mask:0xf bank_mask:0xf bound_ctrl:0\n\t" \
	"v_pk_fma_f32 v[64:65], v[82:83], v[100:101], v[64:65] op_sel:[0,1,0] op_sel_hi:[1,1,1]\n\t" \
	"v_pk_fma_f32 v[66:67], v[90:91], v[100:101], v[66:67] op_sel:[0,1,0] op_sel_hi:[1,1,1]\n\t" \
	"v_pk_fma_f32 v[68:69], v[72:73], v[100:101], v[68:69] op_sel:[0,0,0] op_sel_hi:[1,0,1]\n\t" \
	"v_pk_fma_f32 v[64:65], v[84:85], v[102:103], v[64:65] op_sel:[0,0,0] op_sel_hi:[1,0,1]\n\t" \
	"v_pk_fma_f32 v[66:67], v[92:93], v[102:103], v[66:67] op_sel:[0,0,0] op_sel_hi:[1,0,1]\n\t" \
	"v_pk_fma_f32 v[68:69], v[74:75], v[100:101], v[68:69] op_sel:[0,1,0] op_sel_hi:[1,1,1]\n\t" \
	"v_pk_fma_f32 v[64:65], v[86:87], v[102:103], v[64:65] op_sel:[0,1,0] op_sel_hi:[1,1,1]\n\t" \
	"v_pk_fma_f32 v[66:67], v[94:95], v[102:103], v[66:67] op_sel:[0,1,0] op_sel_hi:[1,1,1]\n\t" \
	"v_pk_fma_f32 v[68:69], v[76:77], v[102:103], v[68:69] op_sel:[0,0,0] op_sel_hi:[1,0,1]\n\t" \
	"s_waitcnt lgkmcnt(3)\n\t" \
	"v_pk_fma_f32 v[64:65], v[88:89], v[104:105], v[64:65] op_sel:[0,0,0] op_sel_hi:[1,0,1]\n\t" \
	"s_bfm_b64 exec, 52, 0\n\t" \
	"v_mov_b32_dpp v66, v66 wave_shr:1 row_mask:0xf bank_mask:0xf bound_ctrl:0\n\t" \
	"v_mov_b32_dpp v67, v67 wave_shr:1 row_mask:0xf bank_mask:0xf bound_ctrl:0\n\t" \
	"s_mov_b64 exec, -1\n\t" \
	"v_pk_fma_f32 v[68:69], v[78:79], v[102:103], v[68:69] op_sel:[0,1,0] op_sel_hi:[1,1,1]\n\t" \
	"v_pk_fma_f32 v[64:65], v[90:91], v[104:105], v[64:65] op_sel:[0,1,0] op_sel_hi:[1,1,1]\n\t" \
	"v_pk_fma_f32 v[66:67], v[72:73], v[104:105], v[66:67] op_sel:[0,0,0] op_sel_hi:[1,0,1]\n\t" \
	"v_pk_fma_f32 v[68:69], v[80:81], v[104:105], v[68:69] op_sel:[0,0,0] op_sel_hi:[1,0,1]\n\t" \
	"v_pk_fma_f32 v[64:65], v[92:93], v[106:107], v[64:65] op_sel:[0,0,0] op_sel_hi:[1,0,1]\n\t" \
	"v_pk_fma_f32 v[66:67], v[74:75], v[104:105], v[66:67] op_sel:[0,1,0] op_sel_hi:[1,1,1]\n\t" \
	"v_pk_fma_f32 v[68:69], v[82:83], v[104:105], v[68:69] op_sel:[0,1,0] op_sel_hi:[1,1,1]\n\t" \
	"v_pk_fma_f32 v[64:65], v[94:95], v[106:107], v[64:65] op_sel:[0,1,0] op_sel_hi:[1,1,1]\n\t" \
	"v_pk_fma_f32 v[66:67], v[76:77], v[106:107], v[66:67] op_sel:[0,0,0] op_sel_hi:[1,0,1]\n\t" \
	"v_pk_fma_f32 v[68:69], v[84:85], v[106:107], v[68:69] op_sel:[0,0,0] op_sel_hi:[1,0,1]\n\t" \
	"v_mov_b32_dpp v64, v64 wave_shr:1 row_mask:0xf bank_mask:0xf bound_ctrl:0\n\t" \
	"v_mov_b32_dpp v65, v65 wave_shr:1 row_mask:0xf bank_mask:0xf bound_ctrl:0\n\t" \
	"v_pk_fma_f32 v[66:67], v[78:79], v[106:107], v[66:67] op_sel:[0,1,0] op_sel_hi:[1,1,1]\n\t" \
	"v_pk_fma_f32 v[68:69], v[86:87], v[106:107], v[68:69] op_sel:[0,1,0] op_sel_hi:[1,1,1]\n\t" \
	"s_waitcnt lgkmcnt(2)\n\t" \
	"v_pk_fma_f32 v[64:65], v[72:73], v[108:109], v[64:65] op_sel:[0,0,0] op_sel_hi:[1,0,1]\n\t" \
	"v_pk_fma_f32 v[66:67], v[80:81], v[108:109], v[66:67] op_sel:[0,0,0] op_sel_hi:[1,0,1]\n\t" \
	"v_pk_fma_f32 v[68:69], v[88:89], v[108:109], v[68:69] op_sel:[0,0,0] op_sel_hi:[1,0,1]\n\t" \
	"v_pk_fma_f32 v[64:65], v[74:75], v[108:109], v[64:65] op_sel:[0,1,0] op_sel_hi:[1,1,1]\n\t" \
	"v_pk_fma_f32 v[66:67], v[82:83], v[108:109], v[66:67] op_sel:[0,1,0] op_sel_hi:[1,1,1]\n\t" \
	"v_pk_fma_f32 v[68:69], v[90:91], v[108:109], v[68:69] op_sel:[0,1,0] op_sel_hi:[1,1,1]\n\t" \
	"v_pk_fma_f32 v[64:65], v[76:77], v[110:111], v[64:65] op_sel:[0,0,0] op_sel_hi:[1,0,1]\n\t" \
	"v_pk_fma_f32 v[66:67], v[84:85], v[110:111], v[66:67] op_sel:[0,0,0] op_sel_hi:[1,0,1]\n\t" \
	"v_pk_fma_f32 v[68:69], v[92:93], v[110:111], v[68:69] op_sel:[0,0,0] op_sel_hi:[1,0,1]\n\t" \
	"v_pk_fma_f32 v[64:65], v[78:79], v[110:111], v[64:65] op_sel:[0,1,0] op_sel_hi:[1,1,1]\n\t" \
	"v_pk_fma_f32 v[66:67], v[86:87], v[110:111], v[66:67] op_sel:[0,1,0] op_sel_hi:[1,1,1]\n\t" \
	"v_pk_fma_f32 v[68:69], v[94:95], v[110:111], v[68:69] op_sel:[0,1,0] op_sel_hi:[1,1,1]\n\t" \
	"s_waitcnt lgkmcnt(1)\n\t" \
	"v_pk_fma_f32 v[64:65], v[80:81], v[124:125], v[64:65] op_sel:[0,0,0] op_sel_hi:[1,0,1]\n\t" \
	"v_pk_fma_f32 v[66:67], v[88:89], v[124:125], v[66:67] op_sel:[0,0,0] op_sel_hi:[1,0,1]\n\t" \
	"v_mov_b32_dpp v68, v68 wave_shr:1 row_mask:0xf bank_mask:0xf bound_ctrl:0\n\t" \
	"v_mov_b32_dpp v69, v69 wave_shr:1 row_mask:0xf bank_mask:0xf bound_ctrl:0\n\t" \
	"v_pk_fma_f32 v[64:65], v[82:83], v[124:125], v[64:65] op_sel:[0,1,0] op_sel_hi:[1,1,1]\n\t" \
	"v_pk_fma_f32 v[66:67], v[90:91], v[124:125], v[66:67] op_sel:[0,1,0] op_sel_hi:[1,1,1]\n\t" \
	"v_pk_fma_f32 v[68:69], v[72:73], v[124:125], v[68:69] op_sel:[0,0,0] op_sel_hi:[1,0,1]\n\t" \
	"v_pk_fma_f32 v[64:65], v[84:85], v[126:127], v[64:65] op_sel:[0,0,0] op_sel_hi:[1,0,1]\n\t" \
	"v_pk_fma_f32 v[66:67], v[92:93], v[126:127], v[66:67] op_sel:[0,0,0] op_sel_hi:[1,0,1]\n\t" \
	"v_pk_fma_f32 v[68:69], v[74:75], v[124:125], v[68:69] op_sel:[0,1,0] op_sel_hi:[1,1,1]\n\t" \
	"v_pk_fma_f32 v[64:65], v[86:87], v[126:127], v[64:65] op_sel:[0,1,0] op_sel_hi:[1,1,1]\n\t" \
	"v_pk_fma_f32 v[66:67], v[94:95], v[126:127], v[66:67] op_sel:[0,1,0] op_sel_hi:[1,1,1]\n\t" \
	"v_pk_fma_f32 v[68:69], v[76:77], v[126:127], v[68:69] op_sel:[0,0,0] op_sel_hi:[1,0,1]\n\t" \
	"s_waitcnt lgkmcnt(0)\n\t" \
	"v_pk_fma_f32 v[64:65], v[88:89], v[120:121], v[64:65] op_sel:[0,0,0] op_sel_hi:[1,0,1]\n\t" \
	"s_bfm_b64 exec, 52, 0\n\t" \
	"v_mov_b32_dpp v66, v66 wave_shr:1 row_mask:0xf bank_mask:0xf bound_ctrl:0\n\t" \
	"v_mov_b32_dpp v67, v67 wave_shr:1 row_mask:0xf bank_mask:0xf bound_ctrl:0\n\t" \
	"s_mov_b64 exec, -1\n\t" \
	"v_pk_fma_f32 v[68:69], v[78:79], v[126:127], v[68:69] op_sel:[0,1,0] op_sel_hi:[1,1,1]\n\t" \
	"v_pk_fma_f32 v[64:65], v[90:91], v[120:121], v[64:65] op_sel:[0,1,0] op_sel_hi:[1,1,1]\n\t" \
	"v_pk_fma_f32 v[66:67], v[72:73], v[120:121], v[66:67] op_sel:[0,0,0] op_sel_hi:[1,0,1]\n\t" \
	"v_pk_fma_f32 v[68:69], v[80:81], v[120:121], v[68:69] op_sel:[0,0,0] op_sel_hi:[1,0,1]\n\t" \
	"v_pk_fma_f32 v[64:65], v[92:93], v[122:123], v[64:65] op_sel:[0,0,0] op_sel_hi:[1,0,1]\n\t" \
	"v_pk_fma_f32 v[66:67], v[74:75], v[120:121], v[66:67] op_sel:[0,1,0] op_sel_hi:[1,1,1]\n\t" \
	"v_pk_fma_f32 v[68:69], v[82:83], v[120:121], v[68:69] op_sel:[0,1,0] op_sel_hi:[1,1,1]\n\t" \
	"v_pk_fma_f32 v[64:65], v[94:95], v[122:123], v[64:65] op_sel:[0,1,0] op_sel_hi:[1,1,1]\n\t" \
	"v_pk_fma_f32 v[66:67], v[76:77], v[122:123], v[66:67] op_sel:[0,0,0] op_sel_hi:[1,0,1]\n\t" \
	"v_pk_fma_f32 v[68:69], v[84:85], v[122:123], v[68:69] op_sel:[0,0,0] op_sel_hi:[1,0,1]\n\t" \
	"v_mov_b32_dpp v64, v64 wave_shr:1 row_mask:0xf bank_mask:0xf bound_ctrl:0\n\t" \
	"v_mov_b32_dpp v65, v65 wave_shr:1 row_mask:0xf bank_mask:0xf bound_ctrl:0\n\t" \
	"v_pk_fma_f32 v[66:67], v[78:79], v[122:123], v[66:67] op_sel:[0,1,0] op_sel_hi:[1,1,1]\n\t" \
	"v_pk_fma_f32 v[68:69], v[86:87], v[122:123], v[68:69] op_sel:[0,1,0] op_sel_hi:[1,1,1]\n\t" \
	"s_mov_b32 exec_lo, 0\n\t" \
	"s_mov_b32 exec_hi, 0xfff00000\n\t" \
	"v_pk_add_f32 v[64:65], v[64:65], v[66:67]\n\t" \
	"s_mov_b64 exec, -1\n\t" \
	"v_mul_f32_dpp %[d1], v119, v66 quad_perm:[3,2,1,0] row_mask:0xf bank_mask:0xf\n\t" \
	"v_mul_f32_dpp %[d2], v119, v68 quad_perm:[0,3,2,1] row_mask:0xf bank_mask:0xf\n\t" \
	"v_mul_f32_dpp %[d0], v119, v64 quad_perm:[2,1,0,3] row_mask:0xf bank_mask:0xf\n\t" \
	"v_fmac_f32_dpp %[d1], v119, v67 quad_perm:[2,1,0,3] row_mask:0xf bank_mask:0xf\n\t" \
	"v_fmac_f32_dpp %[d2], v119, v69 quad_perm:[3,2,1,0] row_mask:0xf bank_mask:0xf\n\t" \
	"v_fmac_f32_dpp %[d0], v119, v65 quad_perm:[1,0,3,2] row_mask:0xf bank_mask:0xf\n\t" \
	".Lnb_tl_end:\n\t"
#define NB_ASM_FIRG \
	"s_ashr_i32 s88, %[nk], 7\n\t" \
	"s_and_b32 s89, %[nk], 127\n\t" \
	"s_lshr_b32 s90, s89, 1\n\t" \
	"s_cmp_ge_u32 s89, 2\n\t" \
	"s_cselect_b32 s90, s90, 64\n\t" \
	"s_sub_u32 s91, -18, s88\n\t" \
	"s_and_b32 s92, s91, 3\n\t" \
	"s_ashr_i32 s93, s91, 2\n\t" \
	"s_mul_i32 s94, s92, 180\n\t" \
	"s_add_u32 s94, s94, s93\n\t" \
	"s_lshl3_add_u32 s94, s94, %[pb]\n\t" \
	"s_mul_i32 s95, s90, 144\n\t" \
	"s_add_u32 s95, s95, %[cb]\n\t" \
	"v_add_u32_e32 v112, s94, %[kic]\n\t" \
	"s_add_u32 s96, s92, 1\n\t" \
	"s_lshr_b32 s96, s96, 2\n\t" \
	"s_mul_i32 s96, s96, -5752\n\t" \
	"s_add_u32 s96, s96, 1440\n\t" \
	"v_add_u32_e32 v113, s96, v112\n\t" \
	"s_add_u32 s96, s92, 2\n\t" \
	"s_lshr_b32 s96, s96, 2\n\t" \
	"s_mul_i32 s96, s96, -5752\n\t" \
	"s_add_u32 s96, s96, 2880\n\t" \
	"v_add_u32_e32 v114, s96, v112\n\t" \
	"s_add_u32 s96, s92, 3\n\t" \
	"s_lshr_b32 s96, s96, 2\n\t" \
	"s_mul_i32 s96, s96, -5752\n\t" \
	"s_add_u32 s96, s96, 4320\n\t" \
	"v_add_u32_e32 v115, s96, v112\n\t" \
	"v_mov_b64_e32 %[a0], 0\n\t" \
	"v_mov_b64_e32 %[a1], 0\n\t" \
	"v_mov_b64_e32 %[a2], 0\n\t" \
	"v_mov_b32_e32 v117, s95\n\t" \
	"s_bfm_b64 exec, 52, 0\n\t" \
	"ds_read_b64 v[72:73], v112 offset:96\n\t" \
	"ds_read_b64 v[74:75], v113 offset:96\n\t" \
	"ds_read_b64 v[76:77], v114 offset:96\n\t" \
	"ds_read_b64 v[78:79], v115 offset:96\n\t" \
	"ds_read_b64 v[80:81], v112 offset:104\n\t" \
	"ds_read_b64 v[82:83], v113 offset:104\n\t" \
	"ds_read_b64 v[84:85], v114 offset:104\n\t" \
	"ds_read_b64 v[86:87], v115 offset:104\n\t" \
	"ds_read_b64 v[88:89], v112 offset:112\n\t" \
	"ds_read_b64 v[90:91], v113 offset:112\n\t" \
	"ds_read_b64 v[92:93], v114 offset:112\n\t" \
	"ds_read_b64 v[94:95], v115 offset:112\n\t" \
	"ds_read_b128 v[104:107], v117\n\t" \
	"ds_read_b128 v[108:111], v117 offset:16\n\t" \
	"ds_read_b64 v[96:97], v112 offset:120\n\t" \
	"ds_read_b64 v[98:99], v113 offset:120\n\t" \
	"ds_read_b64 v[100:101], v114 offset:120\n\t" \
	"ds_read_b64 v[102:103], v115 offset:120\n\t" \
	"s_waitcnt lgkmcnt(5)\n\t" \
	"v_pk_fma_f32 %[a0], v[72:73], v[104:105], %[a0] op_sel:[0,0,0] op_sel_hi:[1,0,1]\n\t" \
	"v_pk_fma_f32 %[a1], v[80:81], v[104:105], %[a1] op_sel:[0,0,0] op_sel_hi:[1,0,1]\n\t" \
	"v_pk_fma_f32 %[a2], v[88:89], v[104:105], %[a2] op_sel:[0,0,0] op_sel_hi:[1,0,1]\n\t" \
	"v_pk_fma_f32 %[a0], v[74:75], v[104:105], %[a0] op_sel:[0,1,0] op_sel_hi:[1,1,1]\n\t" \
	"v_pk_fma_f32 %[a1], v[82:83], v[104:105], %[a1] op_sel:[0,1,0] op_sel_hi:[1,1,1]\n\t" \
	"v_pk_fma_f32 %[a2], v[90:91], v[104:105], %[a2] op_sel:[0,1,0] op_sel_hi:[1,1,1]\n\t" \
	"v_pk_fma_f32 %[a0], v[76:77], v[106:107], %[a0] op_sel:[0,0,0] op_sel_hi:[1,0,1]\n\t" \
	"v_pk_fma_f32 %[a1], v[84:85], v[106:107], %[a1] op_sel:[0,0,0] op_sel_hi:[1,0,1]\n\t" \
	"v_pk_fma_f32 %[a2], v[92:93], v[106:107], %[a2] op_sel:[0,0,0] op_sel_hi:[1,0,1]\n\t" \
	"v_pk_fma_f32 %[a0], v[78:79], v[106:107], %[a0] op_sel:[0,1,0] op_sel_hi:[1,1,1]\n\t" \
	"v_pk_fma_f32 %[a1], v[86:87], v[106:107], %[a1] op_sel:[0,1,0] op_sel_hi:[1,1,1]\n\t" \
	"v_pk_fma_f32 %[a2], v[94:95], v[106:107], %[a2] op_sel:[0,1,0] op_sel_hi:[1,1,1]\n\t" \
	"ds_read_b128 v[104:107], v117 offset:32\n\t" \
	"ds_read_b64 v[72:73], v112 offset:128\n\t" \
	"ds_read_b64 v[74:75], v113 offset:128\n\t" \
	"ds_read_b64 v[76:77], v114 offset:128\n\t" \
	"ds_read_b64 v[78:79], v115 offset:128\n\t" \
	"s_waitcnt lgkmcnt(5)\n\t" \
	"v_pk_fma_f32 %[a0], v[80:81], v[108:109], %[a0] op_sel:[0,0,0] op_sel_hi:[1,0,1]\n\t" \
	"v_pk_fma_f32 %[a1], v[88:89], v[108:109], %[a1] op_sel:[0,0,0] op_sel_hi:[1,0,1]\n\t" \
	"v_pk_fma_f32 %[a2], v[96:97], v[108:109], %[a2] op_sel:[0,0,0] op_sel_hi:[1,0,1]\n\t" \
	"v_pk_fma_f32 %[a0], v[82:83], v[108:109], %[a0] op_sel:[0,1,0] op_sel_hi:[1,1,1]\n\t" \
	"v_pk_fma_f32 %[a1], v[90:91], v[108:109], %[a1] op_sel:[0,1,0] op_sel_hi:[1,1,1]\n\t" \
	"v_pk_fma_f32 %[a2], v[98:99], v[108:109], %[a2] op_sel:[0,1,0] op_sel_hi:[1,1,1]\n\t" \
	"v_pk_fma_f32 %[a0], v[84:85], v[110:111], %[a0] op_sel:[0,0,0] op_sel_hi:[1,0,1]\n\t" \
	"v_pk_fma_f32 %[a1], v[92:93], v[110:111], %[a1] op_sel:[0,0,0] op_sel_hi:[1,0,1]\n\t" \
	"v_pk_fma_f32 %[a2], v[100:101], v[110:111], %[a2] op_sel:[0,0,0] op_sel_hi:[1,0,1]\n\t" \
	"v_pk_fma_f32 %[a0], v[86:87], v[110:111], %[a0] op_sel:[0,1,0] op_sel_hi:[1,1,1]\n\t" \
	"v_pk_fma_f32 %[a1], v[94:95], v[110:111], %[a1] op_sel:[0,1,0] op_sel_hi:[1,1,1]\n\t" \
	"v_pk_fma_f32 %[a2], v[102:103], v[110:111], %[a2] op_sel:[0,1,0] op_sel_hi:[1,1,1]\n\t" \
	"ds_read_b128 v[108:111], v117 offset:48\n\t" \
	"ds_read_b64 v[80:81], v112 offset:136\n\t" \
	"ds_read_b64 v[82:83], v113 offset:136\n\t" \
	"ds_read_b64 v[84:85], v114 offset:136\n\t" \
	"ds_read_b64 v[86:87], v115 offset:136\n\t" \
	"s_waitcnt lgkmcnt(5)\n\t" \
	"v_pk_fma_f32 %[a0], v[88:89], v[104:105], %[a0] op_sel:[0,0,0] op_sel_hi:[1,0,1]\n\t" \
	"v_pk_fma_f32 %[a1], v[96:97], v[104:105], %[a1] op_sel:[0,0,0] op_sel_hi:[1,0,1]\n\t" \
	"v_pk_fma_f32 %[a2], v[72:73], v[104:105], %[a2] op_sel:[0,0,0] op_sel_hi:[1,0,1]\n\t" \
	"v_pk_fma_f32 %[a0], v[90:91], v[104:105], %[a0] op_sel:[0,1,0] op_sel_hi:[1,1,1]\n\t" \
	"v_pk_fma_f32 %[a1], v[98:99], v[104:105], %[a1] op_sel:[0,1,0] op_sel_hi:[1,1,1]\n\t" \
	"v_pk_fma_f32 %[a2], v[74:75], v[104:105], %[a2] op_sel:[0,1,0] op_sel_hi:[1,1,1]\n\t" \
	"v_pk_fma_f32 %[a0], v[92:93], v[106:107], %[a0] op_sel:[0,0,0] op_sel_hi:[1,0,1]\n\t" \
	"v_pk_fma_f32 %[a1], v[100:101], v[106:107], %[a1] op_sel:[0,0,0] op_sel_hi:[1,0,1]\n\t" \
	"v_pk_fma_f32 %[a2], v[76:77], v[106:107], %[a2] op_sel:[0,0,0] op_sel_hi:[1,0,1]\n\t" \
	"v_pk_fma_f32 %[a0], v[94:95], v[106:107], %[a0] op_sel:[0,1,0] op_sel_hi:[1,1,1]\n\t" \
	"v_pk_fma_f32 %[a1], v[102:103], v[106:107], %[a1] op_sel:[0,1,0] op_sel_hi:[1,1,1]\n\t" \
	"v_pk_fma_f32 %[a2], v[78:79], v[106:107], %[a2] op_sel:[0,1,0] op_sel_hi:[1,1,1]\n\t" \
	"ds_read_b128 v[104:107], v117 offset:64\n\t" \
	"ds_read_b64 v[88:89], v112 offset:144\n\t" \
	"ds_read_b64 v[90:91], v113 offset:144\n\t" \
	"ds_read_b64 v[92:93], v114 offset:144\n\t" \
	"ds_read_b64 v[94:95], v115 offset:144\n\t" \
	"s_waitcnt lgkmcnt(5)\n\t" \
	"v_pk_fma_f32 %[a0], v[96:97], v[108:109], %[a0] op_sel:[0,0,0] op_sel_hi:[1,0,1]\n\t" \
	"v_pk_fma_f32 %[a1], v[72:73], v[108:109], %[a1] op_sel:[0,0,0] op_sel_hi:[1,0,1]\n\t" \
	"v_pk_fma_f32 %[a2], v[80:81], v[108:109], %[a2] op_sel:[0,0,0] op_sel_hi:[1,0,1]\n\t" \
	"v_pk_fma_f32 %[a0], v[98:99], v[108:109], %[a0] op_sel:[0,1,0] op_sel_hi:[1,1,1]\n\t" \
	"v_pk_fma_f32 %[a1], v[74:75], v[108:109], %[a1] op_sel:[0,1,0] op_sel_hi:[1,1,1]\n\t" \
	"v_pk_fma_f32 %[a2], v[82:83], v[108:109], %[a2] op_sel:[0,1,0] op_sel_hi:[1,1,1]\n\t" \
	"v_pk_fma_f32 %[a0], v[100:101], v[110:111], %[a0] op_sel:[0,0,0] op_sel_hi:[1,0,1]\n\t" \
	"v_pk_fma_f32 %[a1], v[76:77], v[110:111], %[a1] op_sel:[0,0,0] op_sel_hi:[1,0,1]\n\t" \
	"v_pk_fma_f32 %[a2], v[84:85], v[110:111], %[a2] op_sel:[0,0,0] op_sel_hi:[1,0,1]\n\t" \
	"v_pk_fma_f32 %[a0], v[102:103], v[110:111], %[a0] op_sel:[0,1,0] op_sel_hi:[1,1,1]\n\t" \
	"v_pk_fma_f32 %[a1], v[78:79], v[110:111], %[a1] op_sel:[0,1,0] op_sel_hi:[1,1,1]\n\t" \
	"v_pk_fma_f32 %[a2], v[86:87], v[110:111], %[a2] op_sel:[0,1,0] op_sel_hi:[1,1,1]\n\t" \
	"ds_read_b128 v[108:111], v117 offset:80\n\t" \
	"ds_read_b64 v[96:97], v112 offset:152\n\t" \
	"ds_read_b64 v[98:99], v113 offset:152\n\t" \
	"ds_read_b64 v[100:101], v114 offset:152\n\t" \
	"ds_read_b64 v[102:103], v115 offset:152\n\t" \
	"s_waitcnt lgkmcnt(5)\n\t" \
	"v_pk_fma_f32 %[a0], v[72:73], v[104:105], %[a0] op_sel:[0,0,0] op_sel_hi:[1,0,1]\n\t" \
	"v_pk_fma_f32 %[a1], v[80:81], v[104:105], %[a1] op_sel:[0,0,0] op_sel_hi:[1,0,1]\n\t" \
	"v_pk_fma_f32 %[a2], v[88:89], v[104:105], %[a2] op_sel:[0,0,0] op_sel_hi:[1,0,1]\n\t" \
	"v_pk_fma_f32 %[a0], v[74:75], v[104:105], %[a0] op_sel:[0,1,0] op_sel_hi:[1,1,1]\n\t" \
	"v_pk_fma_f32 %[a1], v[82:83], v[104:105], %[a1] op_sel:[0,1,0] op_sel_hi:[1,1,1]\n\t" \
	"v_pk_fma_f32 %[a2], v[90:91], v[104:105], %[a2] op_sel:[0,1,0] op_sel_hi:[1,1,1]\n\t" \
	"v_pk_fma_f32 %[a0], v[76:77], v[106:107], %[a0] op_sel:[0,0,0] op_sel_hi:[1,0,1]\n\t" \
	"v_pk_fma_f32 %[a1], v[84:85], v[106:107], %[a1] op_sel:[0,0,0] op_sel_hi:[1,0,1]\n\t" \
	"v_pk_fma_f32 %[a2], v[92:93], v[106:107], %[a2] op_sel:[0,0,0] op_sel_hi:[1,0,1]\n\t" \
	"v_pk_fma_f32 %[a0], v[78:79], v[106:107], %[a0] op_sel:[0,1,0] op_sel_hi:[1,1,1]\n\t" \
	"v_pk_fma_f32 %[a1], v[86:87], v[106:107], %[a1] op_sel:[0,1,0] op_sel_hi:[1,1,1]\n\t" \
	"v_pk_fma_f32 %[a2], v[94:95], v[106:107], %[a2] op_sel:[0,1,0] op_sel_hi:[1,1,1]\n\t" \
	"s_waitcnt lgkmcnt(0)\n\t" \
	"v_pk_fma_f32 %[a0], v[80:81], v[108:109], %[a0] op_sel:[0,0,0] op_sel_hi:[1,0,1]\n\t" \
	"v_pk_fma_f32 %[a1], v[88:89], v[108:109], %[a1] op_sel:[0,0,0] op_sel_hi:[1,0,1]\n\t" \
	"v_pk_fma_f32 %[a2], v[96:97], v[108:109], %[a2] op_sel:[0,0,0] op_sel_hi:[1,0,1]\n\t" \
	"v_pk_fma_f32 %[a0], v[82:83], v[108:109], %[a0] op_sel:[0,1,0] op_sel_hi:[1,1,1]\n\t" \
	"v_pk_fma_f32 %[a1], v[90:91], v[108:109], %[a1] op_sel:[0,1,0] op_sel_hi:[1,1,1]\n\t" \
	"v_pk_fma_f32 %[a2], v[98:99], v[108:109], %[a2] op_sel:[0,1,0] op_sel_hi:[1,1,1]\n\t" \
	"v_pk_fma_f32 %[a0], v[84:85], v[110:111], %[a0] op_sel:[0,0,0] op_sel_hi:[1,0,1]\n\t" \
	"v_pk_fma_f32 %[a1], v[92:93], v[110:111], %[a1] op_sel:[0,0,0] op_sel_hi:[1,0,1]\n\t" \
	"v_pk_fma_f32 %[a2], v[100:101], v[110:111], %[a2] op_sel:[0,0,0] op_sel_hi:[1,0,1]\n\t" \
	"v_pk_fma_f32 %[a0], v[86:87], v[110:111], %[a0] op_sel:[0,1,0] op_sel_hi:[1,1,1]\n\t" \
	"v_pk_fma_f32 %[a1], v[94:95], v[110:111], %[a1] op_sel:[0,1,0] op_sel_hi:[1,1,1]\n\t" \
	"v_pk_fma_f32 %[a2], v[102:103], v[110:111], %[a2] op_sel:[0,1,0] op_sel_hi:[1,1,1]\n\t" \
	"s_mov_b64 exec, -1\n\t"
#define NB_ASM_COLD \
	"s_branch .Lnbc_end\n\t" \
	".Lnbc_da_careful:\n\t" \
	"s_mov_b32 s95, 0\n\t" \
	"s_lshl1_add_u32 s96, s95, 0\n\t" \
	"s_bitcmp0_b64 s[90:91], s96\n\t" \
	"s_cbranch_scc1 .Lnbc_da_unsure\n\t" \
	"s_bitcmp1_b64 s[88:89], s96\n\t" \
	"s_addc_u32 s95, s95, s95\n\t" \
	"s_lshl1_add_u32 s96, s95, 2\n\t" \
	"s_bitcmp0_b64 s[90:91], s96\n\t" \
	"s_cbranch_scc1 .Lnbc_da_unsure\n\t" \
	"s_bitcmp1_b64 s[88:89], s96\n\t" \
	"s_addc_u32 s95, s95, s95\n\t" \
	"s_lshl1_add_u32 s96, s95, 6\n\t" \
	"s_bitcmp0_b64 s[90:91], s96\n\t" \
	"s_cbranch_scc1 .Lnbc_da_unsure\n\t" \
	"s_bitcmp1_b64 s[88:89], s96\n\t" \
	"s_addc_u32 s95, s95, s95\n\t" \
	"s_lshl1_add_u32 s96, s95, 14\n\t" \
	"s_bitcmp0_b64 s[90:91], s96\n\t" \
	"s_cbranch_scc1 .Lnbc_da_unsure\n\t" \
	"s_bitcmp1_b64 s[88:89], s96\n\t" \
	"s_addc_u32 s95, s95, s95\n\t" \
	"s_lshl1_add_u32 s96, s95, 30\n\t" \
	"s_bitcmp0_b64 s[90:91], s96\n\t" \
	"s_cbranch_scc1 .Lnbc_da_unsure\n\t" \
	"s_bitcmp1_b64 s[88:89], s96\n\t" \
	"s_addc_u32 s95, s95, s95\n\t" \
	"s_branch .Lnb_da_walked\n\t" \
	".Lnbc_da_unsure:\n\t" \
	"s_mov_b32 s98, 3\n\t" \
	"s_branch .Lnb_da_end\n\t" \
	".Lnbc_da_gate:\n\t" \
	"v_cmp_lt_f32_e32 vcc, v74, v113\n\t" \
	"s_cmp_eq_u64 vcc, 0\n\t" \
	"s_cselect_b32 s98, 2, 0\n\t" \
	"s_mov_b64 exec, -1\n\t" \
	"s_waitcnt lgkmcnt(0)\n\t" \
	"s_branch .Lnb_da_end\n\t" \
	".Lnbc_db_careful:\n\t" \
	"s_mov_b32 s94, 0\n\t" \
	"s_lshl1_add_u32 s95, s94, 0\n\t" \
	"s_bitcmp0_b32 s90, s95\n\t" \
	"s_cbranch_scc1 .Lnbc_db_unsure\n\t" \
	"s_bitcmp1_b32 s88, s95\n\t" \
	"s_addc_u32 s94, s94, s94\n\t" \
	"s_lshl1_add_u32 s95, s94, 2\n\t" \
	"s_bitcmp0_b32 s90, s95\n\t" \
	"s_cbranch_scc1 .Lnbc_db_unsure\n\t" \
	"s_bitcmp1_b32 s88, s95\n\t" \
	"s_addc_u32 s94, s94, s94\n\t" \
	"s_lshl1_add_u32 s95, s94, 6\n\t" \
	"s_bitcmp0_b32 s90, s95\n\t" \
	"s_cbranch_scc1 .Lnbc_db_unsure\n\t" \
	"s_bitcmp1_b32 s88, s95\n\t" \
	"s_addc_u32 s94, s94, s94\n\t" \
	"s_lshl1_add_u32 s95, s94, 14\n\t" \
	"s_bitcmp0_b32 s90, s95\n\t" \
	"s_cbranch_scc1 .Lnbc_db_unsure\n\t" \
	"s_bitcmp1_b32 s88, s95\n\t" \
	"s_addc_u32 s94, s94, s94\n\t" \
	"s_branch .Lnb_db_walked\n\t" \
	".Lnbc_db_unsure:\n\t" \
	"s_mov_b32 s98, 3\n\t" \
	"s_branch .Lnb_db_end\n\t" \
	".Lnbc_tl_wait:\n\t" \
	"s_waitcnt vmcnt(0)\n\t" \
	"s_branch .Lnb_tl_end\n\t" \
	".Lnbc_end:\n\t"
#define NB_ASM_AMAX(FILL0, FILL1, FILL2, FILL3, FILL4, FILL5, FILL6, FILL7) \
	"v_mov_b32_e32 v88, %[nrm]\n\t" \
	"v_mov_b32_dpp v89, %[ep] quad_perm:[0,0,0,0] row_mask:0xf bank_mask:0xf\n\t" \
	FILL0 "\n\t" \
	"v_max_f32_dpp v88, v88, v88 quad_perm:[1,0,3,2] row_mask:0xf bank_mask:0xf\n\t" \
	"v_add_f32_dpp v89, v89, v89 row_half_mirror row_mask:0xf bank_mask:0xf\n\t" \
	FILL1 "\n\t" \
	"v_max_f32_dpp v88, v88, v88 quad_perm:[2,3,0,1] row_mask:0xf bank_mask:0xf\n\t" \
	"v_add_f32_dpp v89, v89, v89 row_mirror row_mask:0xf bank_mask:0xf\n\t" \
	FILL2 "\n\t" \
	"v_max_f32_dpp v88, v88, v88 row_half_mirror row_mask:0xf bank_mask:0xf\n\t" \
	"v_add_f32_dpp v89, v89, v89 row_bcast:15 row_mask:0xa bank_mask:0xf\n\t" \
	FILL3 "\n\t" \
	"v_max_f32_dpp v88, v88, v88 row_mirror row_mask:0xf bank_mask:0xf\n\t" \
	"v_add_f32_dpp v89, v89, v89 row_bcast:31 row_mask:0xc bank_mask:0xf\n\t" \
	FILL4 "\n\t" \
	"v_max_f32_dpp v88, v88, v88 row_bcast:15 row_mask:0xa bank_mask:0xf\n\t" \
	FILL5 "\n\t" \
	"v_readlane_b32 %[es], v89, 63\n\t" \
	"v_max_f32_dpp v88, v88, v88 row_bcast:31 row_mask:0xc bank_mask:0xf\n\t" \
	FILL6 "\n\t" \
	FILL7 "\n\t" \
	"v_readlane_b32 %[m], v88, 63\n\t" \
	"s_nop 1\n\t" \
	"v_cmp_eq_f32_e32 vcc, %[m], %[nrm]\n\t" \
	"s_ff1_i32_b64 %[bidx], vcc\n\t"
```

Before: 1141.

## Fuse peak-refine and demod tail asm blocks, trim scalar ops in detection

Merges the second detection stage and the demodulation tail into one inline-asm block, with a separate tail copy kept for the slow fallback path. This removes the compiler boundary and register hand-off between the two blocks and starts the global load earlier. It also shortens the scalar peak-walk checks (nor plus scc branch instead of or/compare), folds zero-initialised accumulators into the first FMA, and replaces the multiply-based offset arithmetic with selects and immediate LDS offsets. Adds optional memtime diagnostics, but duplicates a large asm block and depends on hand-adjusted LDS offset constants being correct.

```diff
diff --git a/osmo_trx_amd/csrc/trx_kernel_nb.hip b/osmo_trx_amd/csrc/trx_kernel_nb.hip
--- a/osmo_trx_amd/csrc/trx_kernel_nb.hip
+++ b/osmo_trx_amd/csrc/trx_kernel_nb.hip
@@ -1,4 +1,28 @@
 #include "trx_k4_common.h"
+#ifdef TRX_DIAG
+#define NB_DIAG_T(k) NB_DIAG_T##k
+#define NB_DIAG_T0 "s_memtime s[88:89]\n\ts_waitcnt lgkmcnt(0)\n\ts_mov_b32 s99, s88\n\t"
+#define NB_DIAG_T1 "s_memtime s[88:89]\n\ts_waitcnt lgkmcnt(0)\n\ts_sub_u32 s99, s88, s99\n\ts_mov_b32 %[dga], s88\n\t"
+#define NB_DIAG_T2 "s_memtime s[90:91]\n\ts_waitcnt lgkmcnt(0)\n\ts_sub_u32 %[dga], s90, %[dga]\n\t"
+#define NB_DIAG_T3 "s_memtime s[92:93]\n\ts_waitcnt lgkmcnt(0)\n\ts_sub_u32 s91, s92, s90\n\t"
+#define NB_DIAG_T4 "s_memtime s[94:95]\n\ts_waitcnt lgkmcnt(0)\n\ts_sub_u32 s93, s94, s92\n\t" \
+	"s_pack_ll_b32_b16 %[dga], s99, %[dga]\n\ts_pack_ll_b32_b16 %[dgb], s91, s93\n\t"
+#define NB_DIAG_T_DECL unsigned dg_a, dg_b
+#define NB_DIAG_T_OUT , [dga] "=&s"(dg_a), [dgb] "=&s"(dg_b)
+#define NB_DIAG_T_SPLIT                                                                                          \
+	do {                                                                                                     \
+		if (st == 1 && ok) {                                                                             \
+			const unsigned long long _a = dg_a & 0xffffu, _b = dg_a >> 16, _c = dg_b & 0xffffu, _d = dg_b >> 16; \
+			diag_acc[6] += _a; diag_acc[7] += _b; diag_acc[8] += _c; diag_acc[9] += _d;              \
+			diag_acc[10] -= _a + _b + _c + _d;                                                       \
+		}                                                                                                \
+	} while (0)
+#else
+#define NB_DIAG_T(k)
+#define NB_DIAG_T_DECL
+#define NB_DIAG_T_OUT
+#define NB_DIAG_T_SPLIT
+#endif
 #include "trx_nb_asm.inc"
 
 #define NB_D_LEN    160
@@ -101,7 +125,7 @@
 		const int l = threadIdx.x, e = (l - 52) / 3, t = (l - 52) % 3;
 		const bool sp = l >= 52;
 		lcn[3 * WAVE + l] = 8 * (sp ? (t == 0 ? e : t == 1 ? e + 3 : e - 3) : 4 + 3 * (l < 49 ? l : 49));
-		lcn[4 * WAVE + l] = sp ? (e + (t == 2 ? 4 : 0)) * K4_NTP * 4 : -1;
+		lcn[4 * WAVE + l] = sp ? (e + (t == 2 ? 4 : 0)) * K4_NTP * 4 + NB_ASM_AW_D : -1;
 	}
 	for (int i = lane0; i < NB_SLICE; i += WAVE)
 		wbase[i] = make_float2(0.0f, 0.0f);
@@ -414,6 +438,7 @@
 		const unsigned prm0 = (unsigned)uni((int)pre_prm);
 		const unsigned max_toa = prm0 >> 16;
 		const int tsc = (prm0 >> 8) & 0xff;
+		const int t5 = (t5pk << (28 - 4 * tsc)) >> 28;
 #ifdef TRX_DIAG
 		DIAG_MARK(12);
 		asm volatile("s_waitcnt vmcnt(0)" ::: "memory");
@@ -490,12 +515,20 @@
 						     : NB_ASM_CLOBBERS_ST);
 					DIAG_MARK(5);
 					int toa512 = 0, xr_bits = 0, xi_bits = 0;
+					int ok, s_bits;
+					float d0, d1, d2;
 					if (__builtin_expect(st == 1, 1)) {
-						asm volatile(NB_ASM_DETB
-							     : [st] "=&" NB_ASM_ST(st), [toa] "=&s"(toa512), [xr] "=&s"(xr_bits), [xi] "=&s"(xi_bits)
-							     : [e] "s"(e512), [kb] "v"(kb), [czb] "s"(lds_addr(cz)), [km] "v"(km)
+						NB_DIAG_T_DECL;
+						asm volatile(NB_ASM_DETBTAIL
+							     : [st] "=&" NB_ASM_ST(st), [toa] "=&s"(toa512), [xr] "=&s"(xr_bits), [xi] "=&s"(xi_bits),
+							       [ok] "=&s"(ok), [ssum] "=&s"(s_bits), [d0] "=&v"(d0), [d1] "=&v"(d1), [d2] "=&v"(d2) NB_DIAG_T_OUT
+							     : [e] "s"(e512), [kb] "v"(kb), [km] "v"(km), [t5] "s"(t5), [hdrb] "s"(lds_addr(lhdr) + 32u * (unsigned)tsc),
+							       [e8lo] "s"((unsigned)e8_addr), [e8hi] "s"((unsigned)(e8_addr >> 32)), [l16] "v"(a_l16), [aw] "v"(a_w),
+							       [pb] "s"(lds_addr(P)), [cb] "s"(lds_addr(comp) + 4u * (K4_U0 + TRX_FUSED_SH)), [kic] "v"(kic), [ktp] "v"(ktp)
 							     : NB_ASM_CLOBBERS_ST);
-						DIAG_MARK(6);
+						DIAG_MARK(10);
+						NB_DIAG_T_SPLIT;
+						asm volatile("s_setprio 2");
 					}
 					if (__builtin_expect(st != 1, 0)) {
 						int stc = st;
@@ -512,6 +545,14 @@
 							toa512 = uni(toa512);
 							xr_bits = uni(__float_as_int(xcorr.x));
 							xi_bits = uni(__float_as_int(xcorr.y));
+							asm volatile("s_setprio 0");
+							asm volatile(NB_ASM_TAILR
+								     : [ok] "=&s"(ok), [ssum] "=&s"(s_bits), [d0] "=&v"(d0), [d1] "=&v"(d1), [d2] "=&v"(d2)
+								     : [toa] "s"(toa512), [xr] "s"(xr_bits), [xi] "s"(xi_bits), [t5] "s"(t5), [hdrb] "s"(lds_addr(lhdr) + 32u * (unsigned)tsc),
+								       [e8lo] "s"((unsigned)e8_addr), [e8hi] "s"((unsigned)(e8_addr >> 32)), [l16] "v"(a_l16), [aw] "v"(a_w),
+								       [pb] "s"(lds_addr(P)), [cb] "s"(lds_addr(comp) + 4u * (K4_U0 + TRX_FUSED_SH)), [kic] "v"(kic), [ktp] "v"(ktp)
+								     : NB_ASM_CLOBBERS);
+							asm volatile("s_setprio 2");
 							st = 1;
 						} else if (stc == 2) {
 							if (nb_lane_id() == 0) atomicAdd(&g_trx_fast_stats[2], 1ull);
@@ -534,20 +575,8 @@
 							pend_rm = 0xff;
 						}
 					}
+					asm volatile("" : "+s"(st));
 					if (__builtin_expect(st == 1, 1)) {
-						int ok, s_bits;
-						float d0, d1, d2;
-						const int t5 = (t5pk << (28 - 4 * tsc)) >> 28;
-						asm volatile("s_setprio 0");
-						asm volatile(NB_ASM_TAIL
-							     : [ok] "=&s"(ok), [ssum] "=&s"(s_bits), [d0] "=&v"(d0), [d1] "=&v"(d1), [d2] "=&v"(d2)
-							     : [toa] "s"(toa512), [xr] "s"(xr_bits), [xi] "s"(xi_bits), [t5] "s"(t5), [hdrb] "s"(lds_addr(lhdr) + 32u * (unsigned)tsc),
-							       [e8lo] "s"((unsigned)e8_addr), [e8hi] "s"((unsigned)(e8_addr >> 32)), [l16] "v"(a_l16),
-							       [aw] "v"(a_w), [pb] "s"(lds_addr(P)), [cb] "s"(lds_addr(comp) + 4u * (K4_U0 + TRX_FUSED_SH)), [db] "s"(lds_addr(D)),
-							       [kic] "v"(kic), [ktp] "v"(ktp)
-							     : NB_ASM_CLOBBERS);
-						DIAG_MARK(10);
-						asm volatile("s_setprio 2");
 						o.x = __builtin_amdgcn_fmed3f(fmaf(0.5f, d0, 0.5f), 0.0f, 1.0f);
 						o.y = __builtin_amdgcn_fmed3f(fmaf(0.5f, d1, 0.5f), 0.0f, 1.0f);
 						o.z = __builtin_amdgcn_fmed3f(fmaf(0.5f, d2, 0.5f), 0.0f, 1.0f);
diff --git a/osmo_trx_amd/csrc/trx_nb_asm.inc b/osmo_trx_amd/csrc/trx_nb_asm.inc
--- a/osmo_trx_amd/csrc/trx_nb_asm.inc
+++ b/osmo_trx_amd/csrc/trx_nb_asm.inc
@@ -1206,8 +1206,6 @@
 	"ds_read_b64 v[98:99], v66 offset:40\n\t" \
 	"ds_read_b64 v[100:101], v66 offset:48\n\t" \
 	"ds_read_b64 v[102:103], v66 offset:56\n\t" \
-	"v_mov_b64_e32 v[84:85], 0\n\t" \
-	"v_mov_b64_e32 v[86:87], 0\n\t" \
 	"s_add_u32 s91, %[bidx], -1\n\t" \
 	"s_sub_u32 s92, %[len], %[bidx]\n\t" \
 	"s_min_u32 s91, s91, 4\n\t" \
@@ -1244,8 +1242,8 @@
 	"ds_read_b64 v[124:125], v66 offset:112\n\t" \
 	"ds_read_b64 v[126:127], v66 offset:120\n\t" \
 	"s_waitcnt lgkmcnt(10)\n\t" \
-	"v_pk_fma_f32 v[84:85], v[88:89], v[76:77], v[84:85] op_sel:[0,0,0] op_sel_hi:[1,0,1]\n\t" \
-	"v_pk_fma_f32 v[86:87], v[90:91], v[76:77], v[86:87] op_sel:[0,1,0] op_sel_hi:[1,1,1]\n\t" \
+	"v_pk_fma_f32 v[84:85], v[88:89], v[76:77], 0 op_sel:[0,0,0] op_sel_hi:[1,0,0]\n\t" \
+	"v_pk_fma_f32 v[86:87], v[90:91], v[76:77], 0 op_sel:[0,1,0] op_sel_hi:[1,1,0]\n\t" \
 	"v_pk_fma_f32 v[84:85], v[92:93], v[78:79], v[84:85] op_sel:[0,0,0] op_sel_hi:[1,0,1]\n\t" \
 	"v_pk_fma_f32 v[86:87], v[94:95], v[78:79], v[86:87] op_sel:[0,1,0] op_sel_hi:[1,1,1]\n\t" \
 	"v_pk_fma_f32 v[84:85], v[96:97], v[80:81], v[84:85] op_sel:[0,0,0] op_sel_hi:[1,0,1]\n\t" \
@@ -1275,16 +1273,13 @@
 	"v_cmp_lt_f32_e64 s[88:89], v91, v90\n\t" \
 	"s_mov_b32 s98, 1\n\t" \
 	"s_lshr_b64 s[90:91], s[88:89], 1\n\t" \
-	"s_or_b64 s[90:91], s[90:91], s[88:89]\n\t" \
+	"s_nor_b64 s[90:91], s[90:91], s[88:89]\n\t" \
 	"s_mov_b32 s96, 0x55555555\n\t" \
 	"s_mov_b32 s97, 0x15555555\n\t" \
 	"s_and_b64 s[92:93], s[90:91], s[96:97]\n\t" \
-	"s_cmp_eq_u64 s[92:93], s[96:97]\n\t" \
-	"s_cbranch_scc0 .Lnbc_da_careful\n\t" \
-	"s_mov_b32 s95, 0\n\t" \
-	"s_lshl1_add_u32 s96, s95, 0\n\t" \
-	"s_bitcmp1_b64 s[88:89], s96\n\t" \
-	"s_addc_u32 s95, s95, s95\n\t" \
+	"s_cbranch_scc1 .Lnbc_da_careful\n\t" \
+	"s_bitcmp1_b64 s[88:89], 0\n\t" \
+	"s_addc_u32 s95, 0, 0\n\t" \
 	"s_lshl1_add_u32 s96, s95, 2\n\t" \
 	"s_bitcmp1_b64 s[88:89], s96\n\t" \
 	"s_addc_u32 s95, s95, s95\n\t" \
@@ -1302,11 +1297,12 @@
 	"s_add_u32 s94, s94, s95\n\t" \
 	"s_add_u32 %[e], s94, -1008\n\t" \
 	".Lnb_da_end:\n\t"
-#define NB_ASM_DETB \
+#define NB_ASM_DETBTAIL \
+	NB_DIAG_T(0) \
 	"v_mov_b64_e32 v[64:65], 0\n\t" \
 	"v_mov_b64_e32 v[66:67], 0\n\t" \
 	"v_add_u32_e32 v68, %[e], %[kb]\n\t" \
-	"s_add_u32 s88, %[czb], -56\n\t" \
+	"s_add_u32 s88, %[pb], 7080\n\t" \
 	"s_mov_b32 exec_lo, 0x3fffffff\n\t" \
 	"s_mov_b32 exec_hi, 0xffff\n\t" \
 	"v_ashrrev_i32_e32 v69, 9, v68\n\t" \
@@ -1388,14 +1384,11 @@
 	"v_mov_b32_dpp v96, v96 quad_perm:[1,0,3,2] row_mask:0xf bank_mask:0xf\n\t" \
 	"v_cmp_lt_f32_e64 s[88:89], v97, v96\n\t" \
 	"s_lshr_b32 s90, s88, 1\n\t" \
-	"s_or_b32 s90, s90, s88\n\t" \
+	"s_nor_b32 s90, s90, s88\n\t" \
 	"s_and_b32 s91, s90, 0x15555555\n\t" \
-	"s_cmp_eq_u32 s91, 0x15555555\n\t" \
-	"s_cbranch_scc0 .Lnbc_db_careful\n\t" \
-	"s_mov_b32 s94, 0\n\t" \
-	"s_lshl1_add_u32 s95, s94, 0\n\t" \
-	"s_bitcmp1_b32 s88, s95\n\t" \
-	"s_addc_u32 s94, s94, s94\n\t" \
+	"s_cbranch_scc1 .Lnbc_db_careful\n\t" \
+	"s_bitcmp1_b32 s88, 0\n\t" \
+	"s_addc_u32 s94, 0, 0\n\t" \
 	"s_lshl1_add_u32 s95, s94, 2\n\t" \
 	"s_bitcmp1_b32 s88, s95\n\t" \
 	"s_addc_u32 s94, s94, s94\n\t" \
@@ -1410,27 +1403,24 @@
 	"s_lshl1_add_u32 %[toa], s94, s92\n\t" \
 	"v_readlane_b32 %[xr], v74, s93\n\t" \
 	"v_readlane_b32 %[xi], v75, s93\n\t" \
-	".Lnb_db_end:\n\t"
-#define NB_ASM_TAIL \
+	"s_setprio 0\n\t" \
 	"v_mov_b32_e32 v65, %[hdrb]\n\t" \
 	"ds_read_b128 v[68:71], v65\n\t" \
 	"s_sub_u32 s88, %[t5], %[toa]\n\t" \
 	"s_add_u32 s87, s88, 5120\n\t" \
-	"s_mov_b32 %[ok], 0\n\t" \
 	"s_and_b32 s91, s87, 127\n\t" \
-	"s_lshr_b32 s92, s91, 1\n\t" \
+	"s_lshr_b32 s90, s91, 1\n\t" \
 	"s_cmp_ge_u32 s91, 2\n\t" \
-	"s_cselect_b32 s92, s92, 64\n\t" \
-	"s_mul_i32 s93, s92, 768\n\t" \
-	"s_add_u32 s94, %[e8lo], s93\n\t" \
+	"s_cselect_b32 s90, s90, 64\n\t" \
+	"s_mul_i32 s94, s90, 768\n\t" \
+	"s_add_u32 s94, %[e8lo], s94\n\t" \
 	"s_addc_u32 s95, %[e8hi], 0\n\t" \
-	"s_abs_i32 s96, %[toa]\n\t" \
+	"global_load_dwordx4 v[120:123], %[l16], s[94:95]\n\t" \
+	NB_DIAG_T(1) \
+	"s_lshr_b32 s96, %[toa], 31\n\t" \
+	"s_sub_u32 s96, %[toa], s96\n\t" \
 	"s_add_u32 s96, s96, 256\n\t" \
-	"global_load_dwordx4 v[120:123], %[l16], s[94:95]\n\t" \
-	"s_lshr_b32 s96, s96, 9\n\t" \
-	"s_sub_u32 s97, 0, s96\n\t" \
-	"s_cmp_lt_i32 %[toa], 0\n\t" \
-	"s_cselect_b32 s96, s97, s96\n\t" \
+	"s_ashr_i32 s96, s96, 9\n\t" \
 	"s_lshl_b32 s96, s96, 3\n\t" \
 	"v_add_u32_e32 v64, s96, %[aw]\n\t" \
 	"s_bfm_b64 exec, 16, 0\n\t" \
@@ -1451,76 +1441,64 @@
 	"s_mov_b32 s89, 0xaaaaaaaa\n\t" \
 	"v_mul_f32_e32 v91, v86, v89\n\t" \
 	"v_mul_f32_e64 v92, -v87, v89\n\t" \
+	"s_bitreplicate_b64_b32 s[96:97], s88\n\t" \
 	"v_cndmask_b32_e64 v119, v91, v92, s[88:89]\n\t" \
-	"s_mov_b32 s88, 0xcccccccc\n\t" \
-	"s_mov_b32 s89, 0xcccccccc\n\t" \
-	"v_cndmask_b32_e64 v119, v119, -v119, s[88:89]\n\t" \
+	"v_cndmask_b32_e64 v119, v119, -v119, s[96:97]\n\t" \
 	"s_bfm_b64 exec, 16, 0\n\t" \
 	"s_waitcnt lgkmcnt(0)\n\t" \
 	"v_pk_mul_f32 v[66:67], v[66:67], v[66:67]\n\t" \
 	"s_ashr_i32 s88, s87, 7\n\t" \
 	"v_add_f32_e32 v81, v67, v66\n\t" \
-	"s_and_b32 s89, s87, 127\n\t" \
-	"s_lshr_b32 s90, s89, 1\n\t" \
-	"v_add_f32_dpp v81, v81, v81 quad_perm:[1,0,3,2] row_mask:0xf bank_mask:0xf\n\t" \
-	"s_cmp_ge_u32 s89, 2\n\t" \
-	"s_cselect_b32 s90, s90, 64\n\t" \
-	"v_add_f32_dpp v81, v81, v81 quad_perm:[2,3,0,1] row_mask:0xf bank_mask:0xf\n\t" \
 	"s_sub_u32 s91, -18, s88\n\t" \
 	"s_and_b32 s92, s91, 3\n\t" \
-	"v_add_f32_dpp v81, v81, v81 row_half_mirror row_mask:0xf bank_mask:0xf\n\t" \
+	"v_add_f32_dpp v81, v81, v81 quad_perm:[1,0,3,2] row_mask:0xf bank_mask:0xf\n\t" \
 	"s_ashr_i32 s93, s91, 2\n\t" \
 	"s_mul_i32 s94, s92, 180\n\t" \
-	"v_add_f32_dpp v81, v81, v81 row_mirror row_mask:0xf bank_mask:0xf\n\t" \
+	"v_add_f32_dpp v81, v81, v81 quad_perm:[2,3,0,1] row_mask:0xf bank_mask:0xf\n\t" \
 	"s_add_u32 s94, s94, s93\n\t" \
 	"s_lshl3_add_u32 s94, s94, %[pb]\n\t" \
-	"v_mul_f32_e32 v81, 0x3d800000, v81\n\t" \
+	"v_add_f32_dpp v81, v81, v81 row_half_mirror row_mask:0xf bank_mask:0xf\n\t" \
 	"s_mul_i32 s95, s90, 144\n\t" \
 	"s_add_u32 s95, s95, %[cb]\n\t" \
+	"v_add_f32_dpp v81, v81, v81 row_mirror row_mask:0xf bank_mask:0xf\n\t" \
+	"s_sub_u32 s96, 0, s88\n\t" \
+	"v_mul_f32_e32 v81, 0x3d800000, v81\n\t" \
+	"s_cmp_gt_u32 s96, 36\n\t" \
 	"v_readlane_b32 %[ssum], v81, 0\n\t" \
-	"s_mov_b64 exec, -1\n\t" \
-	"s_sub_u32 s96, 0, s88\n\t" \
-	"s_cmp_gt_u32 s96, 36\n\t" \
+	"s_cselect_b32 %[ok], 0, 1\n\t" \
+	"s_mov_b64 exec, -1\n\t" \
 	"s_cbranch_scc1 .Lnbc_tl_wait\n\t" \
-	"s_mov_b32 %[ok], 1\n\t" \
 	"v_add_u32_e32 v112, s94, %[kic]\n\t" \
-	"s_add_u32 s96, s92, 1\n\t" \
-	"s_lshr_b32 s96, s96, 2\n\t" \
-	"s_mul_i32 s96, s96, -5752\n\t" \
-	"s_add_u32 s96, s96, 1440\n\t" \
+	"s_cmp_gt_u32 s92, 2\n\t" \
+	"s_cselect_b32 s96, 0xffffe988, 0\n\t" \
 	"v_add_u32_e32 v113, s96, v112\n\t" \
-	"s_add_u32 s96, s92, 2\n\t" \
-	"s_lshr_b32 s96, s96, 2\n\t" \
-	"s_mul_i32 s96, s96, -5752\n\t" \
-	"s_add_u32 s96, s96, 2880\n\t" \
+	"s_cmp_gt_u32 s92, 1\n\t" \
+	"s_cselect_b32 s96, 0xffffe988, 0\n\t" \
 	"v_add_u32_e32 v114, s96, v112\n\t" \
-	"s_add_u32 s96, s92, 3\n\t" \
-	"s_lshr_b32 s96, s96, 2\n\t" \
-	"s_mul_i32 s96, s96, -5752\n\t" \
-	"s_add_u32 s96, s96, 4320\n\t" \
+	"s_cmp_gt_u32 s92, 0\n\t" \
+	"s_cselect_b32 s96, 0xffffe988, 0\n\t" \
 	"v_add_u32_e32 v115, s96, v112\n\t" \
 	"ds_read_b64 v[72:73], v112 offset:96\n\t" \
-	"ds_read_b64 v[74:75], v113 offset:96\n\t" \
-	"ds_read_b64 v[76:77], v114 offset:96\n\t" \
-	"ds_read_b64 v[78:79], v115 offset:96\n\t" \
+	"ds_read_b64 v[74:75], v113 offset:1536\n\t" \
+	"ds_read_b64 v[76:77], v114 offset:2976\n\t" \
+	"ds_read_b64 v[78:79], v115 offset:4416\n\t" \
 	"ds_read_b64 v[80:81], v112 offset:104\n\t" \
-	"ds_read_b64 v[82:83], v113 offset:104\n\t" \
-	"ds_read_b64 v[84:85], v114 offset:104\n\t" \
-	"ds_read_b64 v[86:87], v115 offset:104\n\t" \
+	"ds_read_b64 v[82:83], v113 offset:1544\n\t" \
+	"ds_read_b64 v[84:85], v114 offset:2984\n\t" \
+	"ds_read_b64 v[86:87], v115 offset:4424\n\t" \
 	"ds_read_b64 v[88:89], v112 offset:112\n\t" \
-	"ds_read_b64 v[90:91], v113 offset:112\n\t" \
-	"ds_read_b64 v[92:93], v114 offset:112\n\t" \
-	"ds_read_b64 v[94:95], v115 offset:112\n\t" \
-	"v_add_u32_e32 v116, %[db], %[l16]\n\t" \
+	"ds_read_b64 v[90:91], v113 offset:1552\n\t" \
+	"ds_read_b64 v[92:93], v114 offset:2992\n\t" \
+	"ds_read_b64 v[94:95], v115 offset:4432\n\t" \
+	"v_add_u32_e32 v116, %[pb], %[l16]\n\t" \
 	"v_cmp_lt_i32_e32 vcc, -1, %[ktp]\n\t" \
-	"v_add_u32_e32 v117, %[db], %[ktp]\n\t" \
+	"v_add_u32_e32 v117, %[pb], %[ktp]\n\t" \
 	"v_mov_b32_e32 v118, s95\n\t" \
-	"v_mov_b64_e32 v[64:65], 0\n\t" \
-	"v_mov_b64_e32 v[66:67], 0\n\t" \
-	"v_mov_b64_e32 v[68:69], 0\n\t" \
 	"v_cndmask_b32_e32 v117, v118, v117, vcc\n\t" \
+	NB_DIAG_T(2) \
 	"s_waitcnt vmcnt(0)\n\t" \
-	"ds_write_b128 v116, v[120:123]\n\t" \
+	NB_DIAG_T(3) \
+	"ds_write_b128 v116, v[120:123] offset:5760\n\t" \
 	"ds_read_b128 v[96:99], v117 offset:0\n\t" \
 	"ds_read_b128 v[100:103], v117 offset:16\n\t" \
 	"ds_read_b128 v[104:107], v117 offset:32\n\t" \
@@ -1528,9 +1506,10 @@
 	"ds_read_b128 v[124:127], v117 offset:64\n\t" \
 	"s_waitcnt lgkmcnt(4)\n\t" \
 	"ds_read_b128 v[120:123], v117 offset:80\n\t" \
-	"v_pk_fma_f32 v[64:65], v[72:73], v[96:97], v[64:65] op_sel:[0,0,0] op_sel_hi:[1,0,1]\n\t" \
-	"v_pk_fma_f32 v[66:67], v[80:81], v[96:97], v[66:67] op_sel:[0,0,0] op_sel_hi:[1,0,1]\n\t" \
-	"v_pk_fma_f32 v[68:69], v[88:89], v[96:97], v[68:69] op_sel:[0,0,0] op_sel_hi:[1,0,1]\n\t" \
+	NB_DIAG_T(4) \
+	"v_pk_fma_f32 v[64:65], v[72:73], v[96:97], 0 op_sel:[0,0,0] op_sel_hi:[1,0,0]\n\t" \
+	"v_pk_fma_f32 v[66:67], v[80:81], v[96:97], 0 op_sel:[0,0,0] op_sel_hi:[1,0,0]\n\t" \
+	"v_pk_fma_f32 v[68:69], v[88:89], v[96:97], 0 op_sel:[0,0,0] op_sel_hi:[1,0,0]\n\t" \
 	"v_pk_fma_f32 v[64:65], v[74:75], v[96:97], v[64:65] op_sel:[0,1,0] op_sel_hi:[1,1,1]\n\t" \
 	"v_pk_fma_f32 v[66:67], v[82:83], v[96:97], v[66:67] op_sel:[0,1,0] op_sel_hi:[1,1,1]\n\t" \
 	"v_pk_fma_f32 v[68:69], v[90:91], v[96:97], v[68:69] op_sel:[0,1,0] op_sel_hi:[1,1,1]\n\t" \
@@ -1632,6 +1611,213 @@
 	"v_fmac_f32_dpp %[d2], v119, v69 quad_perm:[3,2,1,0] row_mask:0xf bank_mask:0xf\n\t" \
 	"v_fmac_f32_dpp %[d0], v119, v65 quad_perm:[1,0,3,2] row_mask:0xf bank_mask:0xf\n\t" \
 	".Lnb_tl_end:\n\t"
+#define NB_ASM_TAILR \
+	"v_mov_b32_e32 v65, %[hdrb]\n\t" \
+	"ds_read_b128 v[68:71], v65\n\t" \
+	"s_sub_u32 s88, %[t5], %[toa]\n\t" \
+	"s_add_u32 s87, s88, 5120\n\t" \
+	"s_and_b32 s91, s87, 127\n\t" \
+	"s_lshr_b32 s90, s91, 1\n\t" \
+	"s_cmp_ge_u32 s91, 2\n\t" \
+	"s_cselect_b32 s90, s90, 64\n\t" \
+	"s_mul_i32 s94, s90, 768\n\t" \
+	"s_add_u32 s94, %[e8lo], s94\n\t" \
+	"s_addc_u32 s95, %[e8hi], 0\n\t" \
+	"global_load_dwordx4 v[120:123], %[l16], s[94:95]\n\t" \
+	"s_lshr_b32 s96, %[toa], 31\n\t" \
+	"s_sub_u32 s96, %[toa], s96\n\t" \
+	"s_add_u32 s96, s96, 256\n\t" \
+	"s_ashr_i32 s96, s96, 9\n\t" \
+	"s_lshl_b32 s96, s96, 3\n\t" \
+	"v_add_u32_e32 v64, s96, %[aw]\n\t" \
+	"s_bfm_b64 exec, 16, 0\n\t" \
+	"ds_read_b64 v[66:67], v64 offset:5760\n\t" \
+	"s_mov_b64 exec, -1\n\t" \
+	"s_waitcnt lgkmcnt(1)\n\t" \
+	"v_mul_f32_e32 v82, %[xr], v70\n\t" \
+	"v_mul_f32_e32 v83, %[xr], v71\n\t" \
+	"v_mul_f32_e32 v84, %[xi], v71\n\t" \
+	"v_mul_f32_e32 v85, %[xi], v70\n\t" \
+	"v_sub_f32_e32 v86, v82, v84\n\t" \
+	"v_add_f32_e32 v87, v83, v85\n\t" \
+	"v_mul_f32_e32 v90, v86, v86\n\t" \
+	"v_mul_f32_e32 v89, v87, v87\n\t" \
+	"v_add_f32_e32 v89, v89, v90\n\t" \
+	"v_rcp_f32_e32 v89, v89\n\t" \
+	"s_mov_b32 s88, 0xaaaaaaaa\n\t" \
+	"s_mov_b32 s89, 0xaaaaaaaa\n\t" \
+	"v_mul_f32_e32 v91, v86, v89\n\t" \
+	"v_mul_f32_e64 v92, -v87, v89\n\t" \
+	"s_bitreplicate_b64_b32 s[96:97], s88\n\t" \
+	"v_cndmask_b32_e64 v119, v91, v92, s[88:89]\n\t" \
+	"v_cndmask_b32_e64 v119, v119, -v119, s[96:97]\n\t" \
+	"s_bfm_b64 exec, 16, 0\n\t" \
+	"s_waitcnt lgkmcnt(0)\n\t" \
+	"v_pk_mul_f32 v[66:67], v[66:67], v[66:67]\n\t" \
+	"s_ashr_i32 s88, s87, 7\n\t" \
+	"v_add_f32_e32 v81, v67, v66\n\t" \
+	"s_sub_u32 s91, -18, s88\n\t" \
+	"s_and_b32 s92, s91, 3\n\t" \
+	"v_add_f32_dpp v81, v81, v81 quad_perm:[1,0,3,2] row_mask:0xf bank_mask:0xf\n\t" \
+	"s_ashr_i32 s93, s91, 2\n\t" \
+	"s_mul_i32 s94, s92, 180\n\t" \
+	"v_add_f32_dpp v81, v81, v81 quad_perm:[2,3,0,1] row_mask:0xf bank_mask:0xf\n\t" \
+	"s_add_u32 s94, s94, s93\n\t" \
+	"s_lshl3_add_u32 s94, s94, %[pb]\n\t" \
+	"v_add_f32_dpp v81, v81, v81 row_half_mirror row_mask:0xf bank_mask:0xf\n\t" \
+	"s_mul_i32 s95, s90, 144\n\t" \
+	"s_add_u32 s95, s95, %[cb]\n\t" \
+	"v_add_f32_dpp v81, v81, v81 row_mirror row_mask:0xf bank_mask:0xf\n\t" \
+	"s_sub_u32 s96, 0, s88\n\t" \
+	"v_mul_f32_e32 v81, 0x3d800000, v81\n\t" \
+	"s_cmp_gt_u32 s96, 36\n\t" \
+	"v_readlane_b32 %[ssum], v81, 0\n\t" \
+	"s_cselect_b32 %[ok], 0, 1\n\t" \
+	"s_mov_b64 exec, -1\n\t" \
+	"s_cbranch_scc1 .Lnbc_tr_wait\n\t" \
+	"v_add_u32_e32 v112, s94, %[kic]\n\t" \
+	"s_cmp_gt_u32 s92, 2\n\t" \
+	"s_cselect_b32 s96, 0xffffe988, 0\n\t" \
+	"v_add_u32_e32 v113, s96, v112\n\t" \
+	"s_cmp_gt_u32 s92, 1\n\t" \
+	"s_cselect_b32 s96, 0xffffe988, 0\n\t" \
+	"v_add_u32_e32 v114, s96, v112\n\t" \
+	"s_cmp_gt_u32 s92, 0\n\t" \
+	"s_cselect_b32 s96, 0xffffe988, 0\n\t" \
+	"v_add_u32_e32 v115, s96, v112\n\t" \
+	"ds_read_b64 v[72:73], v112 offset:96\n\t" \
+	"ds_read_b64 v[74:75], v113 offset:1536\n\t" \
+	"ds_read_b64 v[76:77], v114 offset:2976\n\t" \
+	"ds_read_b64 v[78:79], v115 offset:4416\n\t" \
+	"ds_read_b64 v[80:81], v112 offset:104\n\t" \
+	"ds_read_b64 v[82:83], v113 offset:1544\n\t" \
+	"ds_read_b64 v[84:85], v114 offset:2984\n\t" \
+	"ds_read_b64 v[86:87], v115 offset:4424\n\t" \
+	"ds_read_b64 v[88:89], v112 offset:112\n\t" \
+	"ds_read_b64 v[90:91], v113 offset:1552\n\t" \
+	"ds_read_b64 v[92:93], v114 offset:2992\n\t" \
+	"ds_read_b64 v[94:95], v115 offset:4432\n\t" \
+	"v_add_u32_e32 v116, %[pb], %[l16]\n\t" \
+	"v_cmp_lt_i32_e32 vcc, -1, %[ktp]\n\t" \
+	"v_add_u32_e32 v117, %[pb], %[ktp]\n\t" \
+	"v_mov_b32_e32 v118, s95\n\t" \
+	"v_cndmask_b32_e32 v117, v118, v117, vcc\n\t" \
+	"s_waitcnt vmcnt(0)\n\t" \
+	"ds_write_b128 v116, v[120:123] offset:5760\n\t" \
+	"ds_read_b128 v[96:99], v117 offset:0\n\t" \
+	"ds_read_b128 v[100:103], v117 offset:16\n\t" \
+	"ds_read_b128 v[104:107], v117 offset:32\n\t" \
+	"ds_read_b128 v[108:111], v117 offset:48\n\t" \
+	"ds_read_b128 v[124:127], v117 offset:64\n\t" \
+	"s_waitcnt lgkmcnt(4)\n\t" \
+	"ds_read_b128 v[120:123], v117 offset:80\n\t" \
+	"v_pk_fma_f32 v[64:65], v[72:73], v[96:97], 0 op_sel:[0,0,0] op_sel_hi:[1,0,0]\n\t" \
+	"v_pk_fma_f32 v[66:67], v[80:81], v[96:97], 0 op_sel:[0,0,0] op_sel_hi:[1,0,0]\n\t" \
+	"v_pk_fma_f32 v[68:69], v[88:89], v[96:97], 0 op_sel:[0,0,0] op_sel_hi:[1,0,0]\n\t" \
+	"v_pk_fma_f32 v[64:65], v[74:75], v[96:97], v[64:65] op_sel:[0,1,0] op_sel_hi:[1,1,1]\n\t" \
+	"v_pk_fma_f32 v[66:67], v[82:83], v[96:97], v[66:67] op_sel:[0,1,0] op_sel_hi:[1,1,1]\n\t" \
+	"v_pk_fma_f32 v[68:69], v[90:91], v[96:97], v[68:69] op_sel:[0,1,0] op_sel_hi:[1,1,1]\n\t" \
+	"v_pk_fma_f32 v[64:65], v[76:77], v[98:99], v[64:65] op_sel:[0,0,0] op_sel_hi:[1,0,1]\n\t" \
+	"v_pk_fma_f32 v[66:67], v[84:85], v[98:99], v[66:67] op_sel:[0,0,0] op_sel_hi:[1,0,1]\n\t" \
+	"v_pk_fma_f32 v[68:69], v[92:93], v[98:99], v[68:69] op_sel:[0,0,0] op_sel_hi:[1,0,1]\n\t" \
+	"v_pk_fma_f32 v[64:65], v[78:79], v[98:99], v[64:65] op_sel:[0,1,0] op_sel_hi:[1,1,1]\n\t" \
+	"v_pk_fma_f32 v[66:67], v[86:87], v[98:99], v[66:67] op_sel:[0,1,0] op_sel_hi:[1,1,1]\n\t" \
+	"v_pk_fma_f32 v[68:69], v[94:95], v[98:99], v[68:69] op_sel:[0,1,0] op_sel_hi:[1,1,1]\n\t" \
+	"s_waitcnt lgkmcnt(4)\n\t" \
+	"v_pk_fma_f32 v[64:65], v[80:81], v[100:101], v[64:65] op_sel:[0,0,0] op_sel_hi:[1,0,1]\n\t" \
+	"v_pk_fma_f32 v[66:67], v[88:89], v[100:101], v[66:67] op_sel:[0,0,0] op_sel_hi:[1,0,1]\n\t" \
+	"v_mov_b32_dpp v68, v68 wave_shr:1 row_mask:0xf bank_mask:0xf bound_ctrl:0\n\t" \
+	"v_mov_b32_dpp v69, v69 wave_shr:1 row_mask:0xf bank_mask:0xf bound_ctrl:0\n\t" \
+	"v_pk_fma_f32 v[64:65], v[82:83], v[100:101], v[64:65] op_sel:[0,1,0] op_sel_hi:[1,1,1]\n\t" \
+	"v_pk_fma_f32 v[66:67], v[90:91], v[100:101], v[66:67] op_sel:[0,1,0] op_sel_hi:[1,1,1]\n\t" \
+	"v_pk_fma_f32 v[68:69], v[72:73], v[100:101], v[68:69] op_sel:[0,0,0] op_sel_hi:[1,0,1]\n\t" \
+	"v_pk_fma_f32 v[64:65], v[84:85], v[102:103], v[64:65] op_sel:[0,0,0] op_sel_hi:[1,0,1]\n\t" \
+	"v_pk_fma_f32 v[66:67], v[92:93], v[102:103], v[66:67] op_sel:[0,0,0] op_sel_hi:[1,0,1]\n\t" \
+	"v_pk_fma_f32 v[68:69], v[74:75], v[100:101], v[68:69] op_sel:[0,1,0] op_sel_hi:[1,1,1]\n\t" \
+	"v_pk_fma_f32 v[64:65], v[86:87], v[102:103], v[64:65] op_sel:[0,1,0] op_sel_hi:[1,1,1]\n\t" \
+	"v_pk_fma_f32 v[66:67], v[94:95], v[102:103], v[66:67] op_sel:[0,1,0] op_sel_hi:[1,1,1]\n\t" \
+	"v_pk_fma_f32 v[68:69], v[76:77], v[102:103], v[68:69] op_sel:[0,0,0] op_sel_hi:[1,0,1]\n\t" \
+	"s_waitcnt lgkmcnt(3)\n\t" \
+	"v_pk_fma_f32 v[64:65], v[88:89], v[104:105], v[64:65] op_sel:[0,0,0] op_sel_hi:[1,0,1]\n\t" \
+	"s_bfm_b64 exec, 52, 0\n\t" \
+	"v_mov_b32_dpp v66, v66 wave_shr:1 row_mask:0xf bank_mask:0xf bound_ctrl:0\n\t" \
+	"v_mov_b32_dpp v67, v67 wave_shr:1 row_mask:0xf bank_mask:0xf bound_ctrl:0\n\t" \
+	"s_mov_b64 exec, -1\n\t" \
+	"v_pk_fma_f32 v[68:69], v[78:79], v[102:103], v[68:69] op_sel:[0,1,0] op_sel_hi:[1,1,1]\n\t" \
+	"v_pk_fma_f32 v[64:65], v[90:91], v[104:105], v[64:65] op_sel:[0,1,0] op_sel_hi:[1,1,1]\n\t" \
+	"v_pk_fma_f32 v[66:67], v[72:73], v[104:105], v[66:67] op_sel:[0,0,0] op_sel_hi:[1,0,1]\n\t" \
+	"v_pk_fma_f32 v[68:69], v[80:81], v[104:105], v[68:69] op_sel:[0,0,0] op_sel_hi:[1,0,1]\n\t" \
+	"v_pk_fma_f32 v[64:65], v[92:93], v[106:107], v[64:65] op_sel:[0,0,0] op_sel_hi:[1,0,1]\n\t" \
+	"v_pk_fma_f32 v[66:67], v[74:75], v[104:105], v[66:67] op_sel:[0,1,0] op_sel_hi:[1,1,1]\n\t" \
+	"v_pk_fma_f32 v[68:69], v[82:83], v[104:105], v[68:69] op_sel:[0,1,0] op_sel_hi:[1,1,1]\n\t" \
+	"v_pk_fma_f32 v[64:65], v[94:95], v[106:107], v[64:65] op_sel:[0,1,0] op_sel_hi:[1,1,1]\n\t" \
+	"v_pk_fma_f32 v[66:67], v[76:77], v[106:107], v[66:67] op_sel:[0,0,0] op_sel_hi:[1,0,1]\n\t" \
+	"v_pk_fma_f32 v[68:69], v[84:85], v[106:107], v[68:69] op_sel:[0,0,0] op_sel_hi:[1,0,1]\n\t" \
+	"v_mov_b32_dpp v64, v64 wave_shr:1 row_mask:0xf bank_mask:0xf bound_ctrl:0\n\t" \
+	"v_mov_b32_dpp v65, v65 wave_shr:1 row_mask:0xf bank_mask:0xf bound_ctrl:0\n\t" \
+	"v_pk_fma_f32 v[66:67], v[78:79], v[106:107], v[66:67] op_sel:[0,1,0] op_sel_hi:[1,1,1]\n\t" \
+	"v_pk_fma_f32 v[68:69], v[86:87], v[106:107], v[68:69] op_sel:[0,1,0] op_sel_hi:[1,1,1]\n\t" \
+	"s_waitcnt lgkmcnt(2)\n\t" \
+	"v_pk_fma_f32 v[64:65], v[72:73], v[108:109], v[64:65] op_sel:[0,0,0] op_sel_hi:[1,0,1]\n\t" \
+	"v_pk_fma_f32 v[66:67], v[80:81], v[108:109], v[66:67] op_sel:[0,0,0] op_sel_hi:[1,0,1]\n\t" \
+	"v_pk_fma_f32 v[68:69], v[88:89], v[108:109], v[68:69] op_sel:[0,0,0] op_sel_hi:[1,0,1]\n\t" \
+	"v_pk_fma_f32 v[64:65], v[74:75], v[108:109], v[64:65] op_sel:[0,1,0] op_sel_hi:[1,1,1]\n\t" \
+	"v_pk_fma_f32 v[66:67], v[82:83], v[108:109], v[66:67] op_sel:[0,1,0] op_sel_hi:[1,1,1]\n\t" \
+	"v_pk_fma_f32 v[68:69], v[90:91], v[108:109], v[68:69] op_sel:[0,1,0] op_sel_hi:[1,1,1]\n\t" \
+	"v_pk_fma_f32 v[64:65], v[76:77], v[110:111], v[64:65] op_sel:[0,0,0] op_sel_hi:[1,0,1]\n\t" \
+	"v_pk_fma_f32 v[66:67], v[84:85], v[110:111], v[66:67] op_sel:[0,0,0] op_sel_hi:[1,0,1]\n\t" \
+	"v_pk_fma_f32 v[68:69], v[92:93], v[110:111], v[68:69] op_sel:[0,0,0] op_sel_hi:[1,0,1]\n\t" \
+	"v_pk_fma_f32 v[64:65], v[78:79], v[110:111], v[64:65] op_sel:[0,1,0] op_sel_hi:[1,1,1]\n\t" \
+	"v_pk_fma_f32 v[66:67], v[86:87], v[110:111], v[66:67] op_sel:[0,1,0] op_sel_hi:[1,1,1]\n\t" \
+	"v_pk_fma_f32 v[68:69], v[94:95], v[110:111], v[68:69] op_sel:[0,1,0] op_sel_hi:[1,1,1]\n\t" \
+	"s_waitcnt lgkmcnt(1)\n\t" \
+	"v_pk_fma_f32 v[64:65], v[80:81], v[124:125], v[64:65] op_sel:[0,0,0] op_sel_hi:[1,0,1]\n\t" \
+	"v_pk_fma_f32 v[66:67], v[88:89], v[124:125], v[66:67] op_sel:[0,0,0] op_sel_hi:[1,0,1]\n\t" \
+	"v_mov_b32_dpp v68, v68 wave_shr:1 row_mask:0xf bank_mask:0xf bound_ctrl:0\n\t" \
+	"v_mov_b32_dpp v69, v69 wave_shr:1 row_mask:0xf bank_mask:0xf bound_ctrl:0\n\t" \
+	"v_pk_fma_f32 v[64:65], v[82:83], v[124:125], v[64:65] op_sel:[0,1,0] op_sel_hi:[1,1,1]\n\t" \
+	"v_pk_fma_f32 v[66:67], v[90:91], v[124:125], v[66:67] op_sel:[0,1,0] op_sel_hi:[1,1,1]\n\t" \
+	"v_pk_fma_f32 v[68:69], v[72:73], v[124:125], v[68:69] op_sel:[0,0,0] op_sel_hi:[1,0,1]\n\t" \
+	"v_pk_fma_f32 v[64:65], v[84:85], v[126:127], v[64:65] op_sel:[0,0,0] op_sel_hi:[1,0,1]\n\t" \
+	"v_pk_fma_f32 v[66:67], v[92:93], v[126:127], v[66:67] op_sel:[0,0,0] op_sel_hi:[1,0,1]\n\t" \
+	"v_pk_fma_f32 v[68:69], v[74:75], v[124:125], v[68:69] op_sel:[0,1,0] op_sel_hi:[1,1,1]\n\t" \
+	"v_pk_fma_f32 v[64:65], v[86:87], v[126:127], v[64:65] op_sel:[0,1,0] op_sel_hi:[1,1,1]\n\t" \
+	"v_pk_fma_f32 v[66:67], v[94:95], v[126:127], v[66:67] op_sel:[0,1,0] op_sel_hi:[1,1,1]\n\t" \
+	"v_pk_fma_f32 v[68:69], v[76:77], v[126:127], v[68:69] op_sel:[0,0,0] op_sel_hi:[1,0,1]\n\t" \
+	"s_waitcnt lgkmcnt(0)\n\t" \
+	"v_pk_fma_f32 v[64:65], v[88:89], v[120:121], v[64:65] op_sel:[0,0,0] op_sel_hi:[1,0,1]\n\t" \
+	"s_bfm_b64 exec, 52, 0\n\t" \
+	"v_mov_b32_dpp v66, v66 wave_shr:1 row_mask:0xf bank_mask:0xf bound_ctrl:0\n\t" \
+	"v_mov_b32_dpp v67, v67 wave_shr:1 row_mask:0xf bank_mask:0xf bound_ctrl:0\n\t" \
+	"s_mov_b64 exec, -1\n\t" \
+	"v_pk_fma_f32 v[68:69], v[78:79], v[126:127], v[68:69] op_sel:[0,1,0] op_sel_hi:[1,1,1]\n\t" \
+	"v_pk_fma_f32 v[64:65], v[90:91], v[120:121], v[64:65] op_sel:[0,1,0] op_sel_hi:[1,1,1]\n\t" \
+	"v_pk_fma_f32 v[66:67], v[72:73], v[120:121], v[66:67] op_sel:[0,0,0] op_sel_hi:[1,0,1]\n\t" \
+	"v_pk_fma_f32 v[68:69], v[80:81], v[120:121], v[68:69] op_sel:[0,0,0] op_sel_hi:[1,0,1]\n\t" \
+	"v_pk_fma_f32 v[64:65], v[92:93], v[122:123], v[64:65] op_sel:[0,0,0] op_sel_hi:[1,0,1]\n\t" \
+	"v_pk_fma_f32 v[66:67], v[74:75], v[120:121], v[66:67] op_sel:[0,1,0] op_sel_hi:[1,1,1]\n\t" \
+	"v_pk_fma_f32 v[68:69], v[82:83], v[120:121], v[68:69] op_sel:[0,1,0] op_sel_hi:[1,1,1]\n\t" \
+	"v_pk_fma_f32 v[64:65], v[94:95], v[122:123], v[64:65] op_sel:[0,1,0] op_sel_hi:[1,1,1]\n\t" \
+	"v_pk_fma_f32 v[66:67], v[76:77], v[122:123], v[66:67] op_sel:[0,0,0] op_sel_hi:[1,0,1]\n\t" \
+	"v_pk_fma_f32 v[68:69], v[84:85], v[122:123], v[68:69] op_sel:[0,0,0] op_sel_hi:[1,0,1]\n\t" \
+	"v_mov_b32_dpp v64, v64 wave_shr:1 row_mask:0xf bank_mask:0xf bound_ctrl:0\n\t" \
+	"v_mov_b32_dpp v65, v65 wave_shr:1 row_mask:0xf bank_mask:0xf bound_ctrl:0\n\t" \
+	"v_pk_fma_f32 v[66:67], v[78:79], v[122:123], v[66:67] op_sel:[0,1,0] op_sel_hi:[1,1,1]\n\t" \
+	"v_pk_fma_f32 v[68:69], v[86:87], v[122:123], v[68:69] op_sel:[0,1,0] op_sel_hi:[1,1,1]\n\t" \
+	"s_mov_b32 exec_lo, 0\n\t" \
+	"s_mov_b32 exec_hi, 0xfff00000\n\t" \
+	"v_pk_add_f32 v[64:65], v[64:65], v[66:67]\n\t" \
+	"s_mov_b64 exec, -1\n\t" \
+	"v_mul_f32_dpp %[d1], v119, v66 quad_perm:[3,2,1,0] row_mask:0xf bank_mask:0xf\n\t" \
+	"v_mul_f32_dpp %[d2], v119, v68 quad_perm:[0,3,2,1] row_mask:0xf bank_mask:0xf\n\t" \
+	"v_mul_f32_dpp %[d0], v119, v64 quad_perm:[2,1,0,3] row_mask:0xf bank_mask:0xf\n\t" \
+	"v_fmac_f32_dpp %[d1], v119, v67 quad_perm:[2,1,0,3] row_mask:0xf bank_mask:0xf\n\t" \
+	"v_fmac_f32_dpp %[d2], v119, v69 quad_perm:[3,2,1,0] row_mask:0xf bank_mask:0xf\n\t" \
+	"v_fmac_f32_dpp %[d0], v119, v65 quad_perm:[1,0,3,2] row_mask:0xf bank_mask:0xf\n\t" \
+	"s_branch .Lnbc_tr_end\n\t" \
+	".Lnbc_tr_wait:\n\t" \
+	"s_waitcnt vmcnt(0)\n\t" \
+	".Lnbc_tr_end:\n\t"
 #define NB_ASM_FIRG \
 	"s_ashr_i32 s88, %[nk], 7\n\t" \
 	"s_and_b32 s89, %[nk], 127\n\t" \
@@ -1789,27 +1975,27 @@
 	".Lnbc_da_careful:\n\t" \
 	"s_mov_b32 s95, 0\n\t" \
 	"s_lshl1_add_u32 s96, s95, 0\n\t" \
-	"s_bitcmp0_b64 s[90:91], s96\n\t" \
+	"s_bitcmp1_b64 s[90:91], s96\n\t" \
 	"s_cbranch_scc1 .Lnbc_da_unsure\n\t" \
 	"s_bitcmp1_b64 s[88:89], s96\n\t" \
 	"s_addc_u32 s95, s95, s95\n\t" \
 	"s_lshl1_add_u32 s96, s95, 2\n\t" \
-	"s_bitcmp0_b64 s[90:91], s96\n\t" \
+	"s_bitcmp1_b64 s[90:91], s96\n\t" \
 	"s_cbranch_scc1 .Lnbc_da_unsure\n\t" \
 	"s_bitcmp1_b64 s[88:89], s96\n\t" \
 	"s_addc_u32 s95, s95, s95\n\t" \
 	"s_lshl1_add_u32 s96, s95, 6\n\t" \
-	"s_bitcmp0_b64 s[90:91], s96\n\t" \
+	"s_bitcmp1_b64 s[90:91], s96\n\t" \
 	"s_cbranch_scc1 .Lnbc_da_unsure\n\t" \
 	"s_bitcmp1_b64 s[88:89], s96\n\t" \
 	"s_addc_u32 s95, s95, s95\n\t" \
 	"s_lshl1_add_u32 s96, s95, 14\n\t" \
-	"s_bitcmp0_b64 s[90:91], s96\n\t" \
+	"s_bitcmp1_b64 s[90:91], s96\n\t" \
 	"s_cbranch_scc1 .Lnbc_da_unsure\n\t" \
 	"s_bitcmp1_b64 s[88:89], s96\n\t" \
 	"s_addc_u32 s95, s95, s95\n\t" \
 	"s_lshl1_add_u32 s96, s95, 30\n\t" \
-	"s_bitcmp0_b64 s[90:91], s96\n\t" \
+	"s_bitcmp1_b64 s[90:91], s96\n\t" \
 	"s_cbranch_scc1 .Lnbc_da_unsure\n\t" \
 	"s_bitcmp1_b64 s[88:89], s96\n\t" \
 	"s_addc_u32 s95, s95, s95\n\t" \
@@ -1827,29 +2013,29 @@
 	".Lnbc_db_careful:\n\t" \
 	"s_mov_b32 s94, 0\n\t" \
 	"s_lshl1_add_u32 s95, s94, 0\n\t" \
-	"s_bitcmp0_b32 s90, s95\n\t" \
+	"s_bitcmp1_b32 s90, s95\n\t" \
 	"s_cbranch_scc1 .Lnbc_db_unsure\n\t" \
 	"s_bitcmp1_b32 s88, s95\n\t" \
 	"s_addc_u32 s94, s94, s94\n\t" \
 	"s_lshl1_add_u32 s95, s94, 2\n\t" \
-	"s_bitcmp0_b32 s90, s95\n\t" \
+	"s_bitcmp1_b32 s90, s95\n\t" \
 	"s_cbranch_scc1 .Lnbc_db_unsure\n\t" \
 	"s_bitcmp1_b32 s88, s95\n\t" \
 	"s_addc_u32 s94, s94, s94\n\t" \
 	"s_lshl1_add_u32 s95, s94, 6\n\t" \
-	"s_bitcmp0_b32 s90, s95\n\t" \
+	"s_bitcmp1_b32 s90, s95\n\t" \
 	"s_cbranch_scc1 .Lnbc_db_unsure\n\t" \
 	"s_bitcmp1_b32 s88, s95\n\t" \
 	"s_addc_u32 s94, s94, s94\n\t" \
 	"s_lshl1_add_u32 s95, s94, 14\n\t" \
-	"s_bitcmp0_b32 s90, s95\n\t" \
+	"s_bitcmp1_b32 s90, s95\n\t" \
 	"s_cbranch_scc1 .Lnbc_db_unsure\n\t" \
 	"s_bitcmp1_b32 s88, s95\n\t" \
 	"s_addc_u32 s94, s94, s94\n\t" \
 	"s_branch .Lnb_db_walked\n\t" \
 	".Lnbc_db_unsure:\n\t" \
 	"s_mov_b32 s98, 3\n\t" \
-	"s_branch .Lnb_db_end\n\t" \
+	"s_branch .Lnb_tl_end\n\t" \
 	".Lnbc_tl_wait:\n\t" \
 	"s_waitcnt vmcnt(0)\n\t" \
 	"s_branch .Lnb_tl_end\n\t" \
```

Result: no change. 1152, median of 6 (+0.9%).
